# hypre-space/hypredrive

Measured on NVIDIA B200. Metric: AMG-PCG solve DOF-iters/s, 7pt Poisson 256^3 per GPU, higher is better.
Workload: dtype f64

## Files before the change

### hypredrive_b200/csrc/hdk_amg_setup.cu

```cuda
#include "hdk_amg.cuh"
#include <algorithm>
#include <math.h>
#include <stdlib.h>
#include <time.h>

namespace hdk {

#define C_PT 1
#define F_PT -1
#define SF_PT -3

static double g_t_last = 0.0;
static bool   g_timing = false;
static double wall_now()
{
   struct timespec ts;
   clock_gettime(CLOCK_MONOTONIC, &ts);
   return (double)ts.tv_sec + 1e-9 * (double)ts.tv_nsec;
}
static void stage_mark(const char *name, int level)
{
   if (!g_timing) return;
   cudaStreamSynchronize(g.stream);
   double t = wall_now();
// ... 1640 lines not shown
{
   int i = blockIdx.x * blockDim.x + threadIdx.x;
   if (i >= n) return;
   int    b = rp[i], e = rp[i + 1];
   double d = e > b ? val[b] : 0.0, v;
   if (option == 1)
   {
      v = 0.0;
      for (int k = b; k < e; k++) v = __dadd_rn(v, fabs(val[k]));
      if (orp) for (int k = orp[i]; k < orp[i + 1]; k++) v = __dadd_rn(v, fabs(oval[k]));
      if (d < 0) v = -v;
   }
   else if (option == 4)
   {
      double od = 0.0;
      if (orp) for (int k = orp[i]; k < orp[i + 1]; k++) od = __dadd_rn(od, fabs(oval[k]));
      v = __dadd_rn(fabs(d), __dmul_rn(0.5, od));
      if (v <= (4.0 / 3.0) * fabs(d)) v = fabs(d);
      if (d < 0) v = -v;
   }
   else v = d;
   l1[i] = v;
}

static int relax_l1_option(int type)
{
   if (type == 18) return 1;
   if (type == 8 || type == 13 || type == 14) return 4;
   return 5;
}

static int build_l1(const hdk_csr_s &A, int option, double **out)
{
   int n = A.diag.nrows;
   HDK_TRY(dalloc(out, (size_t)n + 8));
   const int    *orp = A.offd.nnz > 0 ? A.offd.rowptr : nullptr;
   const double *ov  = A.offd.nnz > 0 ? A.offd.val : nullptr;
   k_l1<<<cdiv(n, 256), 256, 0, g.stream>>>(A.diag.rowptr, A.diag.val, orp, ov, n, option, *out);
   HDK_LAUNCH_CHECK();
   return HDK_OK;
}

template <bool FILL>
__global__ void k_lower(const int *rp, const int *col, const double *val, int n, int *cnt, const int *lrp, int *lcol, double *lval)
{
   int i = blockIdx.x * blockDim.x + threadIdx.x;
   if (i > n) return;
   if (i == n) { if (!FILL) cnt[n] = 0; return; }
   int c = 0, p = FILL ? lrp[i] : 0;
   for (int k = rp[i]; k < rp[i + 1]; k++)
      if (col[k] < i) { if (FILL) { lcol[p] = col[k]; lval[p] = val[k]; p++; } else c++; }
   if (!FILL) cnt[i] = c;
}

static int build_lower(const DevCSR &A, DevCSR &L)
{
   int  n = A.nrows;
   int *cnt, *lrp;
   HDK_TRY(dalloc(&cnt, (size_t)n + 1));
   HDK_TRY(dalloc(&lrp, (size_t)n + 1));
   k_lower<false><<<cdiv(n + 1, 256), 256, 0, g.stream>>>(A.rowptr, A.col, A.val, n, cnt, nullptr, nullptr, nullptr);
   HDK_LAUNCH_CHECK();
   HDK_TRY(exclusive_scan_int(cnt, lrp, n + 1));
   int nnz = 0;
   HDK_CUDA(cudaMemcpyAsync(&nnz, lrp + n, sizeof(int), cudaMemcpyDeviceToHost, g.stream));
   HDK_CUDA(cudaStreamSynchronize(g.stream));
   dfree(cnt);
   HDK_TRY(csr_alloc(L, n, n, nnz));
   dfree(L.rowptr); L.rowptr = lrp;
   k_lower<true><<<cdiv(n + 1, 256), 256, 0, g.stream>>>(A.rowptr, A.col, A.val, n, nullptr, lrp, L.col, L.val);
   HDK_LAUNCH_CHECK();
   return csr_analyze(L);
}

__global__ void k_dense_fill(const int *rp, const int *col, const double *val, int n, double *M )
{
   int i = blockIdx.x * blockDim.x + threadIdx.x;
   if (i >= n) return;
   for (int k = rp[i]; k < rp[i + 1]; k++) M[(size_t)i * 2 * n + col[k]] += val[k];
   M[(size_t)i * 2 * n + n + i] = 1.0;
}

__global__ void __launch_bounds__(1024) k_gauss_jordan(double *M, int n, double *inv)
{
   __shared__ double sval[32];
   __shared__ int    sidx[32];
   __shared__ int    piv;
   __shared__ double pivval;
   const int tid = threadIdx.x, nt = blockDim.x, w = 2 * n;
   for (int k = 0; k < n; k++)
   {
      double best = -1.0; int bi = k;
      for (int r = k + tid; r < n; r += nt) { double v = fabs(M[(size_t)r * w + k]); if (v > best) { best = v; bi = r; } }
      for (int o = 16; o > 0; o >>= 1)
      {
         double ov = __shfl_down_sync(0xffffffffu, best, o); int oi = __shfl_down_sync(0xffffffffu, bi, o);
         if (ov > best || (ov == best && oi < bi)) { best = ov; bi = oi; }
      }
      if ((tid & 31) == 0) { sval[tid >> 5] = best; sidx[tid >> 5] = bi; }
      __syncthreads();
      if (tid == 0)
      {
         double b = sval[0]; int i2 = sidx[0];
         for (int q = 1; q < (nt + 31) / 32; q++) if (sval[q] > b || (sval[q] == b && sidx[q] < i2)) { b = sval[q]; i2 = sidx[q]; }
         piv = i2; pivval = M[(size_t)i2 * w + k];
      }
      __syncthreads();
      int    pr = piv;
      double pv = pivval;
      if (pv != 0.0)
      {
         if (pr != k)
            for (int j = tid; j < w; j += nt) { double t = M[(size_t)k * w + j]; M[(size_t)k * w + j] = M[(size_t)pr * w + j]; M[(size_t)pr * w + j] = t; }
         __syncthreads();
         for (int j = tid; j < w; j += nt) M[(size_t)k * w + j] /= pv;
         __syncthreads();
         for (int idx = tid; idx < n * w; idx += nt)
         {
            int r = idx / w, j = idx - r * w;
            if (r != k && j != k)
            {
               double f = M[(size_t)r * w + k];
               if (f != 0.0) M[(size_t)r * w + j] -= f * M[(size_t)k * w + j];
            }
         }
         __syncthreads();
         for (int r = tid; r < n; r += nt) if (r != k) M[(size_t)r * w + k] = 0.0;
      }
      __syncthreads();
   }
   for (int idx = tid; idx < n * n; idx += nt) { int r = idx / n, j = idx - r * n; inv[idx] = M[(size_t)r * w + n + j]; }
}

constexpr int GJ_ONE_CTA = 1024;
__global__ void __launch_bounds__(1024) k_gj_pivot(double *M, int n, int k, double *f)
{
   __shared__ double sval[32];
   __shared__ int    sidx[32];
   __shared__ int    piv;
   __shared__ double pivval;
   const int tid = threadIdx.x, nt = blockDim.x, w = 2 * n;
   double best = -1.0; int bi = k;
   for (int r = k + tid; r < n; r += nt) { double v = fabs(M[(size_t)r * w + k]); if (v > best) { best = v; bi = r; } }
   for (int o = 16; o > 0; o >>= 1)
   {
      double ov = __shfl_down_sync(0xffffffffu, best, o); int oi = __shfl_down_sync(0xffffffffu, bi, o);
      if (ov > best || (ov == best && oi < bi)) { best = ov; bi = oi; }
   }
   if ((tid & 31) == 0) { sval[tid >> 5] = best; sidx[tid >> 5] = bi; }
   __syncthreads();
   if (tid == 0)
   {
      double b = sval[0]; int i2 = sidx[0];
      for (int q = 1; q < (nt + 31) / 32; q++) if (sval[q] > b || (sval[q] == b && sidx[q] < i2)) { b = sval[q]; i2 = sidx[q]; }
      piv = i2; pivval = M[(size_t)i2 * w + k];
   }
   __syncthreads();
   const int    pr = piv;
   const double pv = pivval;
   if (pv != 0.0)
   {
      if (pr != k)
         for (int j = tid; j < w; j += nt) { double t = M[(size_t)k * w + j]; M[(size_t)k * w + j] = M[(size_t)pr * w + j]; M[(size_t)pr * w + j] = t; }
      __syncthreads();
      for (int j = tid; j < w; j += nt) M[(size_t)k * w + j] /= pv;
   }
   for (int r = tid; r < n; r += nt) f[r] = (pv != 0.0 && r != k) ? M[(size_t)r * w + k] : 0.0;
}

__global__ void k_gj_eliminate(double *M, int n, int k, const double *f)
{
   const int    r = blockIdx.y, w = 2 * n;
   const double fr = f[r];
   if (fr == 0.0) return;
   for (int j = k + blockIdx.x * blockDim.x + threadIdx.x; j < w; j += gridDim.x * blockDim.x)
   {
      if (j == k) M[(size_t)r * w + k] = 0.0;
      else M[(size_t)r * w + j] -= fr * M[(size_t)k * w + j];
   }
}

__global__ void k_gj_extract(const double *M, int n, double *inv)
{
   const int64_t idx = blockIdx.x * (int64_t)blockDim.x + threadIdx.x;
   if (idx >= (int64_t)n * n) return;
   const int64_t r = idx / n, j = idx - r * n;
   inv[idx] = M[r * 2 * n + n + j];
}

static int build_dense_inverse(const DevCSR &A, double **inv)
{
   int     n = A.nrows;
   double *M;
   HDK_TRY(dalloc(&M, (size_t)n * 2 * n + 8));
   if (int rc = dalloc(inv, (size_t)n * n + 8)) { dfree(M); return rc; }
   HDK_CUDA(cudaMemsetAsync(M, 0, sizeof(double) * ((size_t)n * 2 * n), g.stream));
   k_dense_fill<<<cdiv(n, 128), 128, 0, g.stream>>>(A.rowptr, A.col, A.val, n, M);
   HDK_LAUNCH_CHECK();
   if (n <= GJ_ONE_CTA)
   {
      k_gauss_jordan<<<1, 1024, 0, g.stream>>>(M, n, *inv);
      HDK_LAUNCH_CHECK();
   }
   else
   {
      double *f;
      if (int rc = dalloc(&f, (size_t)n + 8)) { dfree(M); return rc; }
      for (int k = 0; k < n; k++)
      {
         k_gj_pivot<<<1, 1024, 0, g.stream>>>(M, n, k, f);
         k_gj_eliminate<<<dim3(cdiv(2 * n - k, 256), n), 256, 0, g.stream>>>(M, n, k, f);
      }
      HDK_LAUNCH_CHECK();
      k_gj_extract<<<(unsigned)(((int64_t)n * n + 255) / 256), 256, 0, g.stream>>>(M, n, *inv);
      HDK_LAUNCH_CHECK();
      dfree(f);
   }
   dfree(M);
   return HDK_OK;
}

hdk_csr_s *wrap_local(DevCSR &D, int64_t grows)
{
   hdk_csr_s *A  = new hdk_csr_s();
   A->row_start  = 0; A->row_end = (int64_t)D.nrows - 1; A->global_rows = grows; A->global_nnz = D.nnz;
   A->diag       = D;
   D             = DevCSR();
   return A;
}

void destroy_local(hdk_csr_s *A)
{
   if (!A) return;
   csr_free(A->diag); csr_free(A->offd);
   halo_plan_free(A->halo);
   dfree(A->offd_rows);
   delete A;
}

}

using namespace hdk;

extern "C" {

void hdk_amg_default_params(hdk_amg_params *p)
{
   p->coarsen_type = 8; p->strong_th = 0.25; p->max_row_sum = 0.9;
   p->max_coarse_size = 64; p->min_coarse_size = 0; p->max_levels = 25;
   p->interp_type = 6; p->max_nnz_row = 4; p->trunc_factor = 0.0;
   p->relax_down = 18; p->relax_up = 18; p->relax_coarse = 9;
   p->sweeps_down = p->sweeps_up = p->sweeps_coarse = 1;
   p->relax_weight = p->outer_weight = 1.0;
   p->rand_seed = 2747; p->keep_transpose = 1; p->print_level = 0;
}

int hdk_amg_destroy(hdk_amg *M)
{
   if (!M) return HDK_OK;
   if (g.inited)
   {
      for (auto &L : M->lev)
      {
         if (L.owns_A) destroy_local(L.A);
         destroy_local(L.P); destroy_local(L.R);
         csr_free(L.S); csr_free(L.L);
         dfree(L.cf); dfree(L.measure); dfree(L.f2c);
         if (L.l1_up != L.l1_down) dfree(L.l1_up);
         dfree(L.l1_down);
         dfree(L.u); dfree(L.f); dfree(L.t); dfree(L.gs1); dfree(L.gs2);
         for (int w = 0; w < 2; w++) { dfree(L.dbg_ip[w]); dfree(L.dbg_col[w]); dfree(L.dbg_val[w]); }
      }
      dfree(M->ge_inv); dfree(M->full_f); dfree(M->full_u);
      ipc_gather_free(M->gather);
      for (auto &G : M->graphs) if (G.exec) cudaGraphExecDestroy((cudaGraphExec_t)G.exec);
      M->graphs.clear();
   }
   if (M->tail) hdk_amg_destroy(M->tail);
   delete M;
   return HDK_OK;
}

int finalize_levels(hdk_amg_s *M, const hdk_amg_params *prm, int64_t live_max_rows)
{
   int    rc = HDK_OK;
   double bytes = 0.0;
   for (int l = 0; l < M->nlev && rc == HDK_OK; l++)
   {
      AmgLevel &L = M->lev[(size_t)l];
      int       n = L.n;
      if (live_max_rows >= 0 && n > live_max_rows) continue;
      if ((rc = build_l1(*L.A, relax_l1_option(prm->relax_down), &L.l1_down))) break;
      if (relax_l1_option(prm->relax_up) == relax_l1_option(prm->relax_down)) L.l1_up = L.l1_down;
      else if ((rc = build_l1(*L.A, relax_l1_option(prm->relax_up), &L.l1_up))) break;
      if ((rc = dalloc(&L.t, (size_t)n + 8))) break;
      if (l > 0)
      {
         if ((rc = dalloc(&L.u, (size_t)n + 8))) break;
         if ((rc = dalloc(&L.f, (size_t)n + 8))) break;
      }
      bool tsgs = (prm->relax_down == 11 || prm->relax_down == 12 || prm->relax_up == 11 || prm->relax_up == 12);
      if (tsgs && (rc = build_lower(L.A->diag, L.L))) break;
      if (tsgs && ((rc = dalloc(&L.gs1, (size_t)n + 8)) || (rc = dalloc(&L.gs2, (size_t)n + 8)))) break;
      double nnzA = (double)L.A->diag.nnz + L.A->offd.nnz;
      if (L.P)
      {
         double nnzP = (double)L.P->diag.nnz + L.P->offd.nnz, ncl = (double)L.P->diag.ncols;
         bytes += 24.0 * n;
         bytes += 12.0 * nnzA + 4.0 * (n + 1) + 24.0 * n;
         bytes += 12.0 * nnzP + 4.0 * (ncl + 1) + 8.0 * n + 8.0 * ncl;
         bytes += 12.0 * nnzP + 4.0 * (n + 1) + 16.0 * n + 8.0 * ncl;
         bytes += 12.0 * nnzA + 4.0 * (n + 1) + 32.0 * n;
      }
      else bytes += 8.0 * (double)n * n + 16.0 * n;
   }
   M->vcycle_bytes = bytes;
   return rc;
}

int setup_serial(const hdk_csr_s *A0, const hdk_amg_params *prm, hdk_amg_s **out, bool keep_f2c,
                 int64_t live_max_rows)
{
   hdk_amg_s *M = new hdk_amg_s();
   M->prm       = *prm;
   M->keep_f2c  = keep_f2c;
   M->keep_debug = tune_amg_keep_debug();
   int rc       = HDK_OK;
   M->lev.emplace_back();
   M->lev[0].A = const_cast<hdk_csr_s *>(A0);
   M->lev[0].owns_A = false;
   M->lev[0].n = A0->diag.nrows;
   int  level = 0;
   bool more  = prm->max_levels > 1;
   double nnz0 = (double)A0->diag.nnz + A0->offd.nnz, nnz_sum = nnz0;
   while (more && rc == HDK_OK)
   {
      AmgLevel        &L = M->lev[(size_t)level];
      const hdk_csr_s &A = *L.A;
      int              n = L.n;
      stage_mark(nullptr, level);
      if ((rc = build_strength(A, prm->strong_th, prm->max_row_sum, L.S))) break;
      stage_mark("strength", level);
      if ((rc = dalloc(&L.cf, (size_t)n + 1))) break;
      double *meas, *keep = nullptr;
      if ((rc = dalloc(&meas, (size_t)n + 1))) break;
      if (M->keep_debug) { if ((rc = dalloc(&keep, (size_t)n + 1))) break; }
      L.measure = keep;
      int64_t goff = (level == 0) ? A.row_start : 0;
      rc = run_pmis(L.S, prm->rand_seed, goff, L.cf, meas, keep, nullptr);
      stage_mark("pmis", level);
      dfree(meas);
      if (rc) break;
      int *flag, *f2c;
      if ((rc = dalloc(&flag, (size_t)n + 1))) break;
      if ((rc = dalloc(&f2c, (size_t)n + 1))) break;
      k_cf_flag<<<cdiv(n + 1, 256), 256, 0, g.stream>>>(L.cf, n, flag);
      g.launches++;
      if ((rc = exclusive_scan_int(flag, f2c, n + 1))) break;
      int nc = 0;
      cudaMemcpyAsync(&nc, f2c + n, sizeof(int), cudaMemcpyDeviceToHost, g.stream);
      cudaStreamSynchronize(g.stream);
      dfree(flag);
      if (nc == 0 || nc == n || nc < prm->min_coarse_size) { dfree(f2c); break; }
      DevCSR P, R, C;
      rc = build_interp(A.diag, L.S, L.cf, f2c, nc, prm->max_nnz_row, prm->trunc_factor, P, -1, -1);
      stage_mark("interp", level);
      if (keep_f2c) L.f2c = f2c; else dfree(f2c);
      if (rc) break;
      if ((rc = csr_transpose(P, R))) break;
      stage_mark("transpose", level);
      if ((rc = build_rap(R, A.diag, P, C, -1, -1))) break;
      stage_mark("rap", level);
      C.coarse_op = true;
      if (live_max_rows < 0 || n <= live_max_rows)
      {
         if ((rc = csr_analyze(P))) break;
         if ((rc = csr_analyze(R))) break;
      }
      if (live_max_rows < 0 || nc <= live_max_rows)
      {
         if ((rc = csr_analyze(C))) break;
      }
      stage_mark("analyze", level);
      nnz_sum += C.nnz;
      L.P = wrap_local(P, n);
      L.R = wrap_local(R, nc);
      M->lev.emplace_back();
      AmgLevel &N = M->lev.back();
      N.A = wrap_local(C, nc); N.owns_A = true; N.n = nc;
      level++;
      if (level == prm->max_levels - 1 || nc <= prm->max_coarse_size) more = false;
      if (!M->keep_debug) csr_free(M->lev[(size_t)level - 1].S);
   }
   if (rc == HDK_OK)
   {
      M->nlev = level + 1;
      M->op_complexity = nnz_sum / (nnz0 > 0 ? nnz0 : 1.0);
      rc = finalize_levels(M, prm, live_max_rows);
   }
   if (rc == HDK_OK)
   {
      AmgLevel &Lc = M->lev[(size_t)M->nlev - 1];
      bool      want_ge = (prm->relax_coarse == 9 || prm->relax_coarse == 99 || prm->relax_coarse == 19);
      if (want_ge && (double)Lc.n * Lc.n < 2.0e8 && Lc.n > 0 && Lc.A->offd.nnz == 0)
      {
         rc = build_dense_inverse(Lc.A->diag, &M->ge_inv);
         M->ge_n = Lc.n;
      }
   }
   if (rc == HDK_OK) rc = (cudaStreamSynchronize(g.stream) == cudaSuccess) ? HDK_OK : set_error(HDK_ERR_CUDA, "setup sync failed: %s", cudaGetErrorString(cudaGetLastError()));
   if (rc != HDK_OK) { hdk_amg_destroy(M); return rc; }
   *out = M;
   return HDK_OK;
}

__global__ void k_shift_i64(const int64_t *in, int64_t *out, int64_t n, int64_t shift)
{
   int64_t i = blockIdx.x * (int64_t)blockDim.x + threadIdx.x;
   if (i < n) out[i] = in[i] + shift;
}
__global__ void k_slice_indptr(const int *rp, int r0, int n, int64_t *out)
{
   int i = blockIdx.x * blockDim.x + threadIdx.x;
   if (i <= n) out[i] = (int64_t)rp[r0 + i] - (int64_t)rp[r0];
}
__global__ void k_slice_entries(const int *col, const double *val, int64_t k0, int64_t cnt, int64_t *ocol, double *oval)
{
   int64_t k = blockIdx.x * (int64_t)blockDim.x + threadIdx.x;
   if (k < cnt) { ocol[k] = col[k0 + k]; oval[k] = val[k0 + k]; }
}

static int slice_rows(const DevCSR &D, int r0, int r1, int64_t cs, int64_t ce, int64_t grows, int64_t gcols,
                      bool square, bool distributed, hdk_csr_s **out)
{
   int      n = r1 - r0;
   int      k[2];
   HDK_CUDA(cudaMemcpyAsync(&k[0], D.rowptr + r0, sizeof(int), cudaMemcpyDeviceToHost, g.stream));
   HDK_CUDA(cudaMemcpyAsync(&k[1], D.rowptr + r1, sizeof(int), cudaMemcpyDeviceToHost, g.stream));
   HDK_CUDA(cudaStreamSynchronize(g.stream));
   int64_t  cnt = (int64_t)k[1] - k[0];
   int64_t *ip, *cj;
   double  *va;
   HDK_TRY(dalloc(&ip, (size_t)n + 1));
   HDK_TRY(dalloc(&cj, (size_t)cnt + 1));
   HDK_TRY(dalloc(&va, (size_t)cnt + 1));
   k_slice_indptr<<<cdiv(n + 1, 256), 256, 0, g.stream>>>(D.rowptr, r0, n, ip);
   HDK_LAUNCH_CHECK();
   if (cnt > 0)
   {
      k_slice_entries<<<cdiv(cnt, 256), 256, 0, g.stream>>>(D.col, D.val, k[0], cnt, cj, va);
      HDK_LAUNCH_CHECK();
   }
   int rc = parcsr_build(r0, (int64_t)r1 - 1, cs, ce, grows, gcols, square, distributed, false, ip, cj, va, out);
   dfree(ip); dfree(cj); dfree(va);
   return rc;
}

static int setup_distributed(const hdk_csr_s *A0, const hdk_amg_params *prm, hdk_amg_s **out)
{
   const int R = g.nranks, me = g.rank;
   stage_mark(nullptr, -2);
   if (!A0->orig_indptr) return set_error(HDK_ERR_INVALID, "distributed setup needs the matrix to be built at N > 1");
   std::vector<int64_t> rows_all, nnz_all;
   HDK_TRY(allgather_i64_host(A0->diag.nrows, rows_all));
   HDK_TRY(allgather_i64_host(A0->orig_nnz, nnz_all));
   std::vector<int64_t> roff((size_t)R + 1, 0), koff((size_t)R + 1, 0);
   for (int r = 0; r < R; r++) { roff[(size_t)r + 1] = roff[(size_t)r] + rows_all[(size_t)r]; koff[(size_t)r + 1] = koff[(size_t)r] + nnz_all[(size_t)r]; }
   const int64_t N = roff[(size_t)R], NNZ = koff[(size_t)R];
   if (N > 2000000000LL || NNZ > 2000000000LL)
      return set_error(HDK_ERR_UNSUPPORTED, "global problem (%lld rows, %lld nnz) exceeds the int32 limits of the replicated setup", (long long)N, (long long)NNZ);
   if (roff[(size_t)me] != A0->row_start) return set_error(HDK_ERR_INVALID, "row partition is not contiguous in rank order");
   int64_t *gip, *gcj;
   double  *gva;
   HDK_TRY(dalloc(&gip, (size_t)N + 1));
   HDK_TRY(dalloc(&gcj, (size_t)NNZ + 1));
   HDK_TRY(dalloc(&gva, (size_t)NNZ + 1));
   {
      int64_t n = rows_all[(size_t)me];
      k_shift_i64<<<cdiv(n, 256), 256, 0, g.stream>>>(A0->orig_indptr, gip + roff[(size_t)me], n, koff[(size_t)me]);
      HDK_LAUNCH_CHECK();
      HDK_CUDA(cudaMemcpyAsync(gcj + koff[(size_t)me], A0->orig_cols, sizeof(int64_t) * (size_t)A0->orig_nnz, cudaMemcpyDeviceToDevice, g.stream));
      HDK_CUDA(cudaMemcpyAsync(gva + koff[(size_t)me], A0->orig_vals, sizeof(double) * (size_t)A0->orig_nnz, cudaMemcpyDeviceToDevice, g.stream));
      HDK_CUDA(cudaMemcpyAsync(gip + N, &NNZ, sizeof(int64_t), cudaMemcpyHostToDevice, g.stream));
   }
   for (int r = 0; r < R; r++)
   {
      HDK_TRY(bcast_bytes(gip + roff[(size_t)r], sizeof(int64_t) * (size_t)rows_all[(size_t)r], r));
      HDK_TRY(bcast_bytes(gcj + koff[(size_t)r], sizeof(int64_t) * (size_t)nnz_all[(size_t)r], r));
      HDK_TRY(bcast_bytes(gva + koff[(size_t)r], sizeof(double) * (size_t)nnz_all[(size_t)r], r));
   }
   const int64_t rep_rows = tune_replicate_rows();
   hdk_csr_s *G = nullptr;
   int rc = parcsr_build(0, N - 1, 0, N - 1, N, N, true, false, false, gip, gcj, gva, &G, N <= rep_rows);
   dfree(gip); dfree(gcj); dfree(gva);
   if (rc) return rc;
   stage_mark("gather A", -2);
   hdk_amg_s *Mg = nullptr;
   g_share = !(getenv("HDK_SETUP_SHARE") && atoi(getenv("HDK_SETUP_SHARE")) == 0);
   if (getenv("HDK_SHARE_MIN_ROWS")) g_share_min_rows = atoi(getenv("HDK_SHARE_MIN_ROWS"));
   rc = setup_serial(G, prm, &Mg, true, rep_rows);
   g_share = false;
   if (rc) { destroy_local(G); return rc; }
   Mg->lev[0].owns_A = true;
   stage_mark("global setup", -2);
   const int nl = Mg->nlev;
   std::vector<std::vector<int64_t>> starts((size_t)nl);
   starts[0] = roff;
   int tail_level = nl - 1;
   for (int l = 0; l < nl; l++)
   {
      bool empty = false;
      for (int r = 0; r < R; r++) if (starts[(size_t)l][(size_t)r + 1] <= starts[(size_t)l][(size_t)r]) empty = true;
      if (Mg->lev[(size_t)l].n <= rep_rows || empty) { tail_level = l; break; }
      if (l + 1 < nl)
      {
         std::vector<int64_t> nxt((size_t)R + 1, 0);
         for (int r = 0; r <= R; r++)
         {
            int v = 0;
            HDK_CUDA(cudaMemcpyAsync(&v, Mg->lev[(size_t)l].f2c + starts[(size_t)l][(size_t)r], sizeof(int), cudaMemcpyDeviceToHost, g.stream));
            HDK_CUDA(cudaStreamSynchronize(g.stream));
            nxt[(size_t)r] = v;
         }
         starts[(size_t)l + 1] = nxt;
      }
   }
   hdk_amg_s *M = new hdk_amg_s();
   M->prm = *prm;
   M->tail = Mg; M->tail_level = tail_level;
   M->op_complexity = Mg->op_complexity;
   for (int l = 0; l < tail_level && rc == HDK_OK; l++)
   {
      AmgLevel &Lg = Mg->lev[(size_t)l];
      M->lev.emplace_back();
      AmgLevel &L = M->lev.back();
      const int64_t fs = starts[(size_t)l][(size_t)me], fe = starts[(size_t)l][(size_t)me + 1];
      const int64_t cs = starts[(size_t)l + 1][(size_t)me], ce = starts[(size_t)l + 1][(size_t)me + 1];
      const int64_t nf = Lg.n, nc = Mg->lev[(size_t)l + 1].n;
      L.n = (int)(fe - fs);
      if (l == 0) { L.A = const_cast<hdk_csr_s *>(A0); L.owns_A = false; }
      else
      {
         if ((rc = slice_rows(Lg.A->diag, (int)fs, (int)fe, fs, fe - 1, nf, nf, true, true, &L.A))) break;
         L.owns_A = true;
      }
      if (l + 1 < tail_level)
      {
         if ((rc = slice_rows(Lg.P->diag, (int)fs, (int)fe, cs, ce - 1, nf, nc, false, true, &L.P))) break;
      }
      else
      {
         if ((rc = slice_rows(Lg.P->diag, (int)fs, (int)fe, 0, nc - 1, nf, nc, false, false, &L.P))) break;
      }
      if ((rc = slice_rows(Lg.R->diag, (int)cs, (int)ce, fs, fe - 1, nc, nf, false, true, &L.R))) break;
   }
   stage_mark("slice", -2);
   if (rc == HDK_OK)
   {
      M->nlev = tail_level;
      M->tail_n   = Mg->lev[(size_t)tail_level].n;
      M->tail_off = starts[(size_t)tail_level][(size_t)me];
      M->tail_cnt = starts[(size_t)tail_level][(size_t)me + 1] - M->tail_off;
      rc = finalize_levels(M, prm, -1);
      double vb = M->vcycle_bytes;
      for (int l = tail_level; l < nl; l++)
      {
         AmgLevel &Lg = Mg->lev[(size_t)l];
         double    n = Lg.n, nnzA = Lg.A->diag.nnz;
         if (Lg.P) { double nnzP = Lg.P->diag.nnz, ncl = Lg.P->diag.ncols; vb += 24.0 * n + 2 * (12.0 * nnzA + 4.0 * n) + 56.0 * n + 2 * (12.0 * nnzP) + 28.0 * n + 16.0 * ncl; }
         else vb += 8.0 * n * n + 16.0 * n;
      }
      M->vcycle_bytes = vb;
   }
   if (rc == HDK_OK) rc = dalloc(&M->full_f, (size_t)M->tail_n + 8);
   if (rc == HDK_OK) rc = dalloc(&M->full_u, (size_t)M->tail_n + 8);
   if (rc == HDK_OK)
   {
      for (int l = 0; l < tail_level; l++)
      {
         AmgLevel &Lg = Mg->lev[(size_t)l];
         if (Lg.owns_A) { destroy_local(Lg.A); Lg.A = nullptr; Lg.owns_A = false; }
         destroy_local(Lg.P); Lg.P = nullptr;
         destroy_local(Lg.R); Lg.R = nullptr;
         csr_free(Lg.S); csr_free(Lg.L);
         dfree(Lg.cf); Lg.cf = nullptr; dfree(Lg.measure); Lg.measure = nullptr; dfree(Lg.f2c); Lg.f2c = nullptr;
         if (Lg.l1_up != Lg.l1_down) dfree(Lg.l1_up);
         dfree(Lg.l1_down); Lg.l1_down = Lg.l1_up = nullptr;
         dfree(Lg.u); dfree(Lg.f); dfree(Lg.t); Lg.u = Lg.f = Lg.t = nullptr;
      }
      HDK_CUDA(cudaStreamSynchronize(g.stream));
   }
   stage_mark("finalize", -2);
   if (rc != HDK_OK) { hdk_amg_destroy(M); return rc; }
   *out = M;
   return HDK_OK;
}

int hdk_amg_setup(const hdk_csr *A0, const hdk_amg_params *prm, hdk_amg **out)
{
   HDK_TRY(require_init());
   if (!A0 || !prm || !out) return set_error(HDK_ERR_INVALID, "hdk_amg_setup: null argument");
   if (prm->interp_type != 6) return set_error(HDK_ERR_UNSUPPORTED, "interpolation type %d: only extended+i (6) has a device kernel", prm->interp_type);
   if (prm->trunc_factor < 0.0 || prm->trunc_factor >= 1.0) return set_error(HDK_ERR_INVALID, "interpolation trunc_factor must be in [0, 1)");
   g_timing = getenv("HDK_SETUP_TIMING") && atoi(getenv("HDK_SETUP_TIMING")) == 1;
   const bool replicated = getenv("HDK_SETUP_REPLICATED") && atoi(getenv("HDK_SETUP_REPLICATED")) == 1;
   const bool force_dist = getenv("HDK_SETUP_DIST_FORCE") && atoi(getenv("HDK_SETUP_DIST_FORCE")) == 1;
   if (g.nranks > 1 && replicated) return setup_distributed(A0, prm, out);
   if (g.nranks > 1 || (force_dist && A0->orig_indptr)) return setup_distributed_rows(A0, prm, out);
   return setup_serial(A0, prm, out, false, -1);
}

int hdk_amg_num_levels(const hdk_amg *M) { return M ? M->nlev + (M->tail ? M->tail->nlev - M->tail_level : 0) : 0; }
int hdk_amg_num_dist_levels(const hdk_amg *M) { return (M && M->tail) ? M->nlev : 0; }
double hdk_amg_operator_complexity(const hdk_amg *M) { return M ? M->op_complexity : 0.0; }
double hdk_amg_vcycle_bytes(const hdk_amg *M) { return M ? M->vcycle_bytes : 0.0; }

static const hdk_amg_s *resolve_level(const hdk_amg *M, int &level)
{
   if (M && M->tail && level >= M->nlev) { level = level - M->nlev + M->tail_level; return M->tail; }
   return M;
}

int hdk_amg_level_info(const hdk_amg *M, int level, int64_t *rows, int64_t *nnz_A, int64_t *nnz_P)
{
   M = resolve_level(M, level);
   if (!M || level < 0 || level >= M->nlev) return set_error(HDK_ERR_INVALID, "level out of range");
   const AmgLevel &L = M->lev[(size_t)level];
   if (rows) *rows = L.n;
   if (nnz_A) *nnz_A = (int64_t)L.A->diag.nnz + L.A->offd.nnz;
   if (nnz_P) *nnz_P = L.P ? L.P->diag.nnz : 0;
   return HDK_OK;
}

int hdk_amg_get_matrix(const hdk_amg *M, int level, int which, int32_t *rowptr_h, int32_t *col_h, double *val_h)
{
   HDK_TRY(require_init());
   M = resolve_level(M, level);
   if (!M || level < 0 || level >= M->nlev) return set_error(HDK_ERR_INVALID, "level out of range");
   const AmgLevel &L = M->lev[(size_t)level];
   const DevCSR   *D = nullptr;
   if (which == 0) D = &L.A->diag;
   else if (which == 1 && L.P) D = &L.P->diag;
   else if (which == 2 && L.R) D = &L.R->diag;
   else if (which == 3 && L.S.rowptr) D = &L.S;
   if (!D) return set_error(HDK_ERR_INVALID, "matrix %d not available on level %d", which, level);
   if (rowptr_h) HDK_CUDA(cudaMemcpyAsync(rowptr_h, D->rowptr, sizeof(int) * ((size_t)D->nrows + 1), cudaMemcpyDeviceToHost, g.stream));
   if (col_h && D->nnz) HDK_CUDA(cudaMemcpyAsync(col_h, D->col, sizeof(int) * (size_t)D->nnz, cudaMemcpyDeviceToHost, g.stream));
   if (val_h && D->val && D->nnz) HDK_CUDA(cudaMemcpyAsync(val_h, D->val, sizeof(double) * (size_t)D->nnz, cudaMemcpyDeviceToHost, g.stream));
   HDK_CUDA(cudaStreamSynchronize(g.stream));
   return HDK_OK;
}

static int get_level_array(const hdk_amg *M, int level, const void *src, size_t bytes, void *dst)
{
   HDK_TRY(require_init());
   if (!M || level < 0 || level >= M->nlev || !src) return set_error(HDK_ERR_INVALID, "array not available on level %d", level);
   return hdk_copy_d2h(dst, src, bytes);
}
int hdk_amg_get_cf(const hdk_amg *M, int level, int32_t *cf_h)
{
   M = resolve_level(M, level);
   if (!M || level < 0 || level >= M->nlev) return set_error(HDK_ERR_INVALID, "level out of range");
   return get_level_array(M, level, M->lev[(size_t)level].cf, sizeof(int) * (size_t)M->lev[(size_t)level].n, cf_h);
}
int hdk_amg_get_measure(const hdk_amg *M, int level, double *m_h)
{
   M = resolve_level(M, level);
   if (!M || level < 0 || level >= M->nlev) return set_error(HDK_ERR_INVALID, "level out of range");
   return get_level_array(M, level, M->lev[(size_t)level].measure, sizeof(double) * (size_t)M->lev[(size_t)level].n, m_h);
}
int hdk_amg_get_l1(const hdk_amg *M, int level, double *l1_h)
{
   M = resolve_level(M, level);
   if (!M || level < 0 || level >= M->nlev) return set_error(HDK_ERR_INVALID, "level out of range");
   return get_level_array(M, level, M->lev[(size_t)level].l1_down, sizeof(double) * (size_t)M->lev[(size_t)level].n, l1_h);
}

int hdk_amg_strength(const hdk_csr *A, double theta, double max_row_sum, int64_t *nnz_S, int32_t **rowptr_d, int32_t **col_d)
{
   HDK_TRY(require_init());
   if (!A) return set_error(HDK_ERR_INVALID, "null matrix");
   DevCSR S;
   HDK_TRY(build_strength(*A, theta, max_row_sum, S));
   *nnz_S = S.nnz; *rowptr_d = S.rowptr; *col_d = S.col;
   return HDK_OK;
}

int hdk_amg_pmis(int64_t n, const int32_t *S_rowptr_d, const int32_t *S_col_d, int seed, int64_t global_offset,
                 int32_t *cf_d, double *measure_d, int *iterations)
{
   HDK_TRY(require_init());
   DevCSR S;
   S.nrows = (int)n; S.ncols = (int)n; S.rowptr = const_cast<int *>(S_rowptr_d); S.col = const_cast<int *>(S_col_d);
   HDK_CUDA(cudaMemcpyAsync(&S.nnz, S_rowptr_d + n, sizeof(int), cudaMemcpyDeviceToHost, g.stream));
   HDK_CUDA(cudaStreamSynchronize(g.stream));
   double *work;
   HDK_TRY(dalloc(&work, (size_t)n + 1));
   int rc = run_pmis(S, seed, global_offset, cf_d, work, measure_d, iterations);
   dfree(work);
   return rc;
}

}
```

### hypredrive_b200/csrc/hdk_amg_solve.cu

```cuda
#include "hdk_amg.cuh"

namespace hdk {

__global__ void __launch_bounds__(256) k_dense_apply(const double *__restrict__ Ainv, const double *__restrict__ f,
                                                     double *__restrict__ u, int n)
{
   int row = blockIdx.x * 8 + (threadIdx.x >> 5), lane = threadIdx.x & 31;
   if (row >= n) return;
   double acc = 0.0;
   for (int j = lane; j < n; j += 32) acc += Ainv[(size_t)row * n + j] * f[j];
   acc = warp_sum(acc);
   if (lane == 0) u[row] = acc;
}

static bool is_jacobi(int t) { return t == 18 || t == 7 || t == 0; }

static int relax_sweep(hdk_amg_s *M, int l, int type, const double *l1, const double *f, const double *in,
                       double *out, int fin, double *fin_out, const hdk_csr_s *export_to = nullptr)
{
   AmgLevel &L = M->lev[(size_t)l];
   SpmvArgs  a;
   a.x = in; a.y = out; a.b = f; a.d = l1; a.w = M->prm.relax_weight;
   if (is_jacobi(type))
   {
// ... 59 lines not shown
      HDK_LAUNCH_CHECK();
      return HDK_OK;
   }
   int     type = (M->prm.relax_coarse == 9 || M->prm.relax_coarse == 99) ? 18 : M->prm.relax_coarse;
   double *cur = u, *oth = alt;
   int     sweeps = M->prm.sweeps_coarse < 1 ? 1 : M->prm.sweeps_coarse;
   for (int s = 0; s < sweeps; s++)
   {
      if (s == 0 && zero_guess && is_jacobi(type))
      {
         HDK_TRY(vec_scaled_div(cur, f, L.l1_down, M->prm.relax_weight, L.n));
      }
      else
      {
         if (s == 0 && zero_guess) HDK_TRY(vec_fill(cur, 0.0, L.n));
         HDK_TRY(relax_sweep(M, l, type, L.l1_down, f, cur, oth, FIN_NONE, nullptr));
         double *tmp = cur; cur = oth; oth = tmp;
      }
   }
   *result = cur;
   return HDK_OK;
}

static double *cycle_start_buffer(hdk_amg_s *M, int l0, double *u0, bool zero_guess)
{
   const hdk_amg_params &p = M->prm;
   const int nfine = M->tail ? M->nlev : M->nlev - 1;
   int       oop;
   if (nfine <= l0) oop = 0;
   else
   {
      int down_oop = zero_guess && is_jacobi(p.relax_down) ? (p.sweeps_down > 0 ? p.sweeps_down - 1 : 0) : p.sweeps_down;
      oop          = down_oop + p.sweeps_up;
   }
   const bool start_in_u0 = zero_guess ? (oop % 2 == 0) : true;
   return start_in_u0 ? u0 : M->lev[(size_t)l0].t;
}

static int amg_cycle_impl(hdk_amg_s *M, const double *f0, double *u0, bool zero_guess, int fin, double *fin_out, int l0, int kg);

static int first_graph_level(hdk_amg_s *M, int l0)
{
   if (M->tail || M->graph_off) return -1;
   const int64_t rows = tune_graph_rows();
   if (rows <= 0) return -1;
   const hdk_amg_params &p = M->prm;
   if (!is_jacobi(p.relax_down) || !is_jacobi(p.relax_up)) return -1;
   for (int l = l0; l < M->nlev; l++)
      if (M->lev[(size_t)l].n <= rows) return l;
   return -1;
}

static int cycle_graph_run(hdk_amg_s *M, const double *f, double *u, bool zero_guess, bool prefilled, int kg)
{
   for (auto &G : M->graphs)
      if (G.f == f && G.u == u && G.zero_guess == zero_guess && G.prefilled == prefilled && G.level == kg)
      {
         HDK_CUDA(cudaGraphLaunch((cudaGraphExec_t)G.exec, g.stream));
         g.launches += G.nodes;
         return HDK_OK;
      }
   const int64_t before = g.launches;
   cudaGraph_t   graph = nullptr;
   if (cudaStreamBeginCapture(g.stream, cudaStreamCaptureModeThreadLocal) != cudaSuccess)
   {
      cudaGetLastError();
      M->graph_off = true;
      M->prefilled_at = prefilled ? kg : -1;
      return amg_cycle_impl(M, f, u, zero_guess, FIN_NONE, nullptr, kg, -1);
   }
   M->prefilled_at = prefilled ? kg : -1;
   int         rc = amg_cycle_impl(M, f, u, zero_guess, FIN_NONE, nullptr, kg, -1);
   cudaError_t e = cudaStreamEndCapture(g.stream, &graph);
   cudaGraphExec_t exec = nullptr;
   if (rc == HDK_OK && e == cudaSuccess && graph) e = cudaGraphInstantiate(&exec, graph, 0);
   if (graph) cudaGraphDestroy(graph);
   if (rc != HDK_OK || e != cudaSuccess || !exec)
   {
      cudaGetLastError();
      M->graph_off = true;
      if (rc != HDK_OK) return rc;
      M->prefilled_at = prefilled ? kg : -1;
      return amg_cycle_impl(M, f, u, zero_guess, FIN_NONE, nullptr, kg, -1);
   }
   hdk_amg_s::CycleGraph G;
   G.f = f; G.u = u; G.zero_guess = zero_guess; G.prefilled = prefilled; G.level = kg; G.exec = exec;
   G.nodes = (int)(g.launches - before);
   g.launches = before;
   M->graphs.push_back(G);
   HDK_CUDA(cudaGraphLaunch(exec, g.stream));
   g.launches += G.nodes;
   return HDK_OK;
}

int amg_cycle(hdk_amg_s *M, const double *f0, double *u0, bool zero_guess, int fin, double *fin_out, int l0)
{
   int kg = first_graph_level(M, l0);
   if (kg == l0)
   {
      if (fin == FIN_NONE)
      {
         const bool pf = (M->prefilled_at == l0) && zero_guess;
         M->prefilled_at = -1;
         return cycle_graph_run(M, f0, u0, zero_guess, pf, l0);
      }
      kg = (l0 + 1 < M->nlev) ? l0 + 1 : -1;
   }
   return amg_cycle_impl(M, f0, u0, zero_guess, fin, fin_out, l0, kg);
}

static int amg_cycle_impl(hdk_amg_s *M, const double *f0, double *u0, bool zero_guess, int fin, double *fin_out, int l0, int kg)
{
   const int             nl = M->nlev;
   const bool            has_tail = (M->tail != nullptr);
   const int             nfine = has_tail ? nl : nl - 1;
   const hdk_amg_params &p = M->prm;
   std::vector<double *> cur((size_t)nl + 1, nullptr), alt((size_t)nl + 1, nullptr);
   std::vector<const double *> rhs((size_t)nl + 1, nullptr);
   bool                  fin_done = false;
   if (has_tail && nl == 0)
   {
      HDK_TRY(vec_fill(M->full_f, 0.0, M->tail_n));
      HDK_TRY(vec_copy(M->full_f + M->tail_off, f0, M->tail_cnt));
      HDK_TRY(allreduce_dev(M->full_f, (int)M->tail_n));
      if (!zero_guess)
      {
         HDK_TRY(vec_fill(M->full_u, 0.0, M->tail_n));
         HDK_TRY(vec_copy(M->full_u + M->tail_off, u0, M->tail_cnt));
         HDK_TRY(allreduce_dev(M->full_u, (int)M->tail_n));
      }
      HDK_TRY(amg_cycle(M->tail, M->full_f, M->full_u, zero_guess, FIN_NONE, nullptr, M->tail_level));
      HDK_TRY(vec_copy(u0, M->full_u + M->tail_off, M->tail_cnt));
      if (fin != FIN_NONE) HDK_TRY(vec_dot_dev(f0, u0, M->tail_cnt, fin, fin_out));
      return HDK_OK;
   }
   {
      AmgLevel &L0 = M->lev[(size_t)l0];
      cur[(size_t)l0] = cycle_start_buffer(M, l0, u0, zero_guess);
      alt[(size_t)l0] = (cur[(size_t)l0] == u0) ? L0.t : u0;
      rhs[(size_t)l0] = f0;
   }
   for (int l = l0 + 1; l < nl; l++) { cur[(size_t)l] = M->lev[(size_t)l].u; alt[(size_t)l] = M->lev[(size_t)l].t; rhs[(size_t)l] = M->lev[(size_t)l].f; }

   bool prefilled = (M->prefilled_at == l0) && zero_guess;
   M->prefilled_at = -1;
   const bool sub = (kg > l0 && kg < nl);
   const int  ndown = sub ? kg : nfine;
   if (sub) cur[(size_t)kg] = cycle_start_buffer(M, kg, M->lev[(size_t)kg].u, true);
   for (int l = l0; l < ndown; l++)
   {
      AmgLevel &L = M->lev[(size_t)l];
      bool      zg = (l > l0) || zero_guess;
      for (int s = 0; s < p.sweeps_down; s++)
      {
         if (s == 0 && zg && is_jacobi(p.relax_down))
         {
            tl_mark(l, 5);
            if (!prefilled) HDK_TRY(vec_scaled_div(cur[(size_t)l], rhs[(size_t)l], L.l1_down, p.relax_weight, L.n, L.A));
         }
         else
         {
            tl_mark(l, 10);
            if (s == 0 && zg) HDK_TRY(vec_fill(cur[(size_t)l], 0.0, L.n));
            HDK_TRY(relax_sweep(M, l, p.relax_down, L.l1_down, rhs[(size_t)l], cur[(size_t)l], alt[(size_t)l], FIN_NONE, nullptr, L.A));
            std::swap(cur[(size_t)l], alt[(size_t)l]);
         }
      }
      if (p.sweeps_down == 0 && zg) HDK_TRY(vec_fill(cur[(size_t)l], 0.0, L.n));
      if (p.sweeps_down == 0 && zg)
      {
         HDK_TRY(vec_copy(alt[(size_t)l], rhs[(size_t)l], L.n));
      }
      else
      {
         SpmvArgs a;
         a.x = cur[(size_t)l]; a.y = alt[(size_t)l]; a.b = rhs[(size_t)l];
         a.export_to = L.R;
         tl_mark(l, 1);
         HDK_TRY(parcsr_matvec(*L.A, SPMV_RESIDUAL, a));
      }
      SpmvArgs rr;
      tl_mark(l, 2);
      rr.x = alt[(size_t)l];
      prefilled = false;
      if (l + 1 < nl) rr.y = M->lev[(size_t)l + 1].f;
      else
      {
         if (M->gather.on) rr.y = ipc_gather_buffer(M->gather) + M->tail_off;
         else
         {
            HDK_TRY(vec_fill(M->full_f, 0.0, M->tail_n));
            rr.y = M->full_f + M->tail_off;
         }
      }
      if (l + 1 < nfine && p.sweeps_down > 0 && is_jacobi(p.relax_down))
      {
         rr.y2 = cur[(size_t)l + 1]; rr.d = M->lev[(size_t)l + 1].l1_down; rr.w = p.relax_weight;
         if (!(sub && l + 1 == kg)) { rr.export_to = M->lev[(size_t)l + 1].A; rr.export_y2 = true; }
         HDK_TRY(parcsr_matvec(*L.R, SPMV_SET_DIV, rr));
         prefilled = true;
      }
      else HDK_TRY(parcsr_matvec(*L.R, SPMV_SET, rr));
   }
   const double *coarse_sol = nullptr;
   tl_mark(ndown, 6);
   if (sub)
   {
      AmgLevel &Lk = M->lev[(size_t)kg];
      HDK_TRY(cycle_graph_run(M, Lk.f, Lk.u, true, prefilled, kg));
      cur[(size_t)kg] = Lk.u;
   }
   else if (has_tail)
   {
      const double *tf = M->full_f;
      if (M->gather.on)
      {
         HDK_TRY(ipc_gather(M->gather, M->tail_off, M->tail_cnt));
         tf = M->gather.buf[M->gather.seq & 1];
      }
      else HDK_TRY(allreduce_dev(M->full_f, (int)M->tail_n));
      HDK_TRY(amg_cycle(M->tail, tf, M->full_u, true, FIN_NONE, nullptr, M->tail_level));
      coarse_sol = M->full_u;
   }
   else
   {
      const int Lc = nl - 1;
      double   *res;
      bool      zg = (Lc > l0) || zero_guess;
      HDK_TRY(coarse_solve(M, Lc, rhs[(size_t)Lc], cur[(size_t)Lc], alt[(size_t)Lc], zg, &res));
      if (res != cur[(size_t)Lc]) std::swap(cur[(size_t)Lc], alt[(size_t)Lc]);
      coarse_sol = cur[(size_t)Lc];
   }
   for (int l = ndown - 1; l >= l0; l--)
   {
      AmgLevel &L = M->lev[(size_t)l];
      tl_mark(l, 3);
      SpmvArgs a;
      a.x = (l + 1 < nl) ? cur[(size_t)l + 1] : coarse_sol;
      a.y = cur[(size_t)l];
      if (p.sweeps_up > 0) a.export_to = L.A;
      else if (l > l0) a.export_to = M->lev[(size_t)l - 1].P;
      HDK_TRY(parcsr_matvec(*L.P, SPMV_ADD, a));
      for (int s = 0; s < p.sweeps_up; s++)
      {
         bool last = (l == l0 && s == p.sweeps_up - 1);
         int  f_   = (last && fin != FIN_NONE) ? fin : FIN_NONE;
         const hdk_csr_s *next = (s + 1 < p.sweeps_up) ? L.A : (l > l0 ? M->lev[(size_t)l - 1].P : nullptr);
         tl_mark(l, 4);
         HDK_TRY(relax_sweep(M, l, p.relax_up, L.l1_up, rhs[(size_t)l], cur[(size_t)l], alt[(size_t)l], f_, fin_out, next));
         std::swap(cur[(size_t)l], alt[(size_t)l]);
         if (f_ != FIN_NONE) fin_done = true;
      }
   }
   tl_mark(l0, 0);
   if (cur[(size_t)l0] != u0) HDK_TRY(vec_copy(u0, cur[(size_t)l0], M->lev[(size_t)l0].n));
   if (fin != FIN_NONE && !fin_done) HDK_TRY(vec_dot_dev(f0, u0, M->lev[(size_t)l0].n, fin, fin_out));
   return HDK_OK;
}

bool amg_prefill_target(hdk_amg_s *M, double *z, double **buf, const double **d, double *w, const hdk_csr_s **reader)
{
   if (reader) *reader = (M->nlev > 0) ? M->lev[0].A : nullptr;
   const hdk_amg_params &p = M->prm;
   const bool has_tail = (M->tail != nullptr);
   const int  nl = M->nlev, nfine = has_tail ? nl : nl - 1;
   if (nl == 0 || nfine <= 0 || p.sweeps_down <= 0 || !is_jacobi(p.relax_down)) return false;
   const int  oop = (p.sweeps_down - 1) + p.sweeps_up;
   *buf = (oop % 2 == 0) ? z : M->lev[0].t;
   *d   = M->lev[0].l1_down;
   *w   = p.relax_weight;
   return true;
}

int amg_precond(hdk_amg_s *M, const double *r, double *z, int fin, double *fin_out)
{
   return amg_cycle(M, r, z, true, fin, fin_out, 0);
}

}

using namespace hdk;

extern "C" {

int hdk_amg_apply(hdk_amg *M, const double *r_d, double *z_d)
{
   HDK_TRY(require_init());
   if (!M) return set_error(HDK_ERR_INVALID, "null hierarchy");
   return amg_precond(M, r_d, z_d, FIN_NONE, nullptr);
}

int hdk_amg_vcycle(hdk_amg *M, const double *f_d, double *u_d)
{
   HDK_TRY(require_init());
   if (!M) return set_error(HDK_ERR_INVALID, "null hierarchy");
   return amg_cycle(M, f_d, u_d, false, FIN_NONE, nullptr, 0);
}

int hdk_time_kernel(const hdk_csr *A, hdk_amg *M, int kernel, int reps, double *avg_ms, double *bytes)
{
   HDK_TRY(require_init());
   if (!A) return set_error(HDK_ERR_INVALID, "null matrix");
   const int64_t n = A->diag.nrows;
   const double  nnz = (double)A->diag.nnz + A->offd.nnz;
   double *x, *y, *b, *d, *z;
   HDK_TRY(dalloc(&x, (size_t)n + 8)); HDK_TRY(dalloc(&y, (size_t)n + 8));
   HDK_TRY(dalloc(&b, (size_t)n + 8)); HDK_TRY(dalloc(&d, (size_t)n + 8));
   HDK_TRY(dalloc(&z, (size_t)n + 8));
   HDK_TRY(hdk_vec_random(x, n, A->row_start, 1));
   HDK_TRY(hdk_vec_random(b, n, A->row_start, 2));
   HDK_TRY(vec_fill(d, 6.0, n));
   HDK_TRY(vec_fill(y, 0.0, n));
   double by = 0.0;
   int    rc = HDK_OK;
   for (int pass = 0; pass < 2 && rc == HDK_OK; pass++)
   {
      int count = pass == 0 ? 3 : reps;
      if (pass == 1) HDK_CUDA(cudaEventRecord(g.ev_a, g.stream));
      for (int it = 0; it < count && rc == HDK_OK; it++)
      {
         SpmvArgs a;
         a.x = x; a.y = y; a.b = b; a.d = d;
         switch (kernel)
         {
            case 0: rc = parcsr_matvec(*A, SPMV_SET, a); by = 12.0 * nnz + 4.0 * (n + 1) + 16.0 * n; break;
            case 1: rc = parcsr_matvec(*A, SPMV_JACOBI, a); by = 12.0 * nnz + 4.0 * (n + 1) + 32.0 * n; break;
            case 2: rc = parcsr_matvec(*A, SPMV_RESIDUAL, a); by = 12.0 * nnz + 4.0 * (n + 1) + 24.0 * n; break;
            case 3:
               rc = vec_fill(g.dscal + S_ALPHA, 1e-3, 1);
               if (rc == HDK_OK) rc = pcg_update_xr(y, b, x, d, n, g.dscal, FIN_IPROD, nullptr, z, d, 1.0);
               by = 64.0 * n; break;
            case 5:
               rc = vec_fill(g.dscal + S_BETA, 0.5, 1);
               if (rc == HDK_OK) rc = pcg_update_p(y, x, n, g.dscal);
               by = 24.0 * n; break;
            case 4:
               if (!M) rc = set_error(HDK_ERR_INVALID, "V-cycle timing needs a hierarchy");
               else { rc = amg_precond(M, b, y, FIN_NONE, nullptr); by = M->vcycle_bytes; }
               break;
            case 6:
               if (!M || M->nlev < 1 || !M->lev[0].L.rowptr) rc = set_error(HDK_ERR_INVALID, "two-stage GS timing needs a hierarchy set up with relaxation 11 or 12");
               else
               {
                  const int    type = (M->prm.relax_down == 12 || M->prm.relax_up == 12) ? 12 : 11;
                  const double nnzL = (double)M->lev[0].L.nnz;
                  rc = relax_sweep(M, 0, type, M->lev[0].l1_down, b, x, y, FIN_NONE, nullptr);
                  by = 12.0 * nnz + 4.0 * (n + 1) + 40.0 * n + (type == 11 ? 1 : 2) * (12.0 * nnzL + 4.0 * (n + 1) + 32.0 * n) + (type == 12 ? 8.0 * n : 0.0);
               }
               break;
            case 7: rc = halo_exchange_begin(*A, x); by = 8.0 * A->halo.n_send; break;
            case 8:
               dbg_skip_exchange(true);
               rc = parcsr_matvec(*A, SPMV_SET, a); by = 12.0 * nnz + 4.0 * (n + 1) + 16.0 * n;
               dbg_skip_exchange(false);
               break;
            default: rc = set_error(HDK_ERR_INVALID, "unknown kernel id %d", kernel);
         }
      }
   }
   if (rc == HDK_OK)
   {
      HDK_CUDA(cudaEventRecord(g.ev_b, g.stream));
      HDK_CUDA(cudaEventSynchronize(g.ev_b));
      float ms = 0.f;
      HDK_CUDA(cudaEventElapsedTime(&ms, g.ev_a, g.ev_b));
      if (avg_ms) *avg_ms = (double)ms / (reps > 0 ? reps : 1);
      if (bytes) *bytes = by;
   }
   dfree(x); dfree(y); dfree(b); dfree(d); dfree(z);
   return rc;
}

}
```

### hypredrive_b200/csrc/hdk_csr.cu

```cuda
#include "hdk_internal.cuh"
#include <cub/cub.cuh>

namespace hdk {

__global__ void k_split_count(const int64_t *indptr, const int64_t *cols, int nrows, int64_t rs,
                              int64_t re, int *cnt_d, int *cnt_o)
{
   int r = blockIdx.x * blockDim.x + threadIdx.x;
   if (r > nrows) return;
   if (r == nrows) { cnt_d[r] = 0; cnt_o[r] = 0; return; }
   int cd = 0, co = 0;
   for (int64_t k = indptr[r]; k < indptr[r + 1]; k++)
   {
      int64_t c = cols[k];
      if (c >= rs && c <= re) cd++; else co++;
   }
   cnt_d[r] = cd; cnt_o[r] = co;
}

__global__ void k_split_fill(const int64_t *indptr, const int64_t *cols, const double *vals, int nrows,
                             int64_t rs, int64_t re, const int *rp_d, int *col_d, double *val_d,
                             const int *rp_o, int64_t *gcol_o, double *val_o, int square)
{
   int r = blockIdx.x * blockDim.x + threadIdx.x;
// ... 304 lines not shown
   return HDK_OK;
}

__global__ void k_offd_correct(const int *rows, const int *rowptr, const int *col, const double *val, int nrows,
                               const double *xh, double *y, const double *d, double w, int mode,
                               double alpha, const double *dotv, const double *diag_part,
                               double *dot_out, double *partials, unsigned *ticket)
{
   __shared__ double red[128 / 32];
   __shared__ int    lastflag;
   double            dcorr = 0.0;
   int i = blockIdx.x * blockDim.x + threadIdx.x;
   if (i < nrows)
   {
      int r = rows[i];
      int s = rowptr[r], e = rowptr[r + 1];
      double acc = 0.0;
      for (int k = s; k < e; k++) acc += val[k] * __ldcg(xh + col[k]);
      double delta = 0.0;
      switch (mode)
      {
         case SPMV_SET:
         case SPMV_ADD: delta = acc; break;
         case SPMV_AXPBY: delta = alpha * acc; break;
         case SPMV_RESIDUAL: delta = -acc; break;
         case SPMV_JACOBI:
         case SPMV_JACOBI_R: { double dd = d[r]; if (dd != 0.0) delta = -(w * acc) / dd; break; }
      }
      y[r] += delta;
      if (dotv) dcorr = dotv[r] * delta;
   }
   if (dotv)
   {
      double bs = block_sum<128>(dcorr, red);
      if (threadIdx.x == 0)
      {
         partials[blockIdx.x] = bs;
         __threadfence();
         unsigned t = atomicInc(ticket, gridDim.x - 1);
         lastflag   = (t == gridDim.x - 1);
      }
      __syncthreads();
      if (lastflag)
      {
         __threadfence();
         double sacc = 0.0;
         for (unsigned b = threadIdx.x; b < gridDim.x; b += 128) sacc += __ldcg(partials + b);
         __syncthreads();
         sacc = block_sum<128>(sacc, red);
         if (threadIdx.x == 0) *dot_out = *diag_part + sacc;
      }
   }
}

__device__ __forceinline__ void grid_xyz(int64_t row, int nx, int ny, int &gx, int &gy, int &gz)
{
   gx = (int)(row % nx);
   int64_t t = row / nx;
   gy = (int)(t % ny);
   gz = (int)(t / ny);
}

__device__ __forceinline__ double axial_velocity(double y, double z, double Hy, double Hz, double umax)
{
   return 16.0 * umax * (y / Hy) * (1.0 - y / Hy) * (z / Hz) * (1.0 - z / Hz);
}

__global__ void k_stencil_count(int kind, int nx, int ny, int nz, int64_t rs, int nrows, int64_t *cnt)
{
   int i = blockIdx.x * blockDim.x + threadIdx.x;
   if (i > nrows) return;
   if (i == nrows) { cnt[i] = 0; return; }
   int gx, gy, gz;
   grid_xyz(rs + i, nx, ny, gx, gy, gz);
   int c;
   if (kind == 27)
   {
      int ax = 1 + (gx > 0) + (gx < nx - 1), ay = 1 + (gy > 0) + (gy < ny - 1), az = 1 + (gz > 0) + (gz < nz - 1);
      c = ax * ay * az;
   }
   else c = 1 + (gx > 0) + (gx < nx - 1) + (gy > 0) + (gy < ny - 1) + (gz > 0) + (gz < nz - 1);
   cnt[i] = c;
}

__global__ void k_stencil_fill(int kind, int nx, int ny, int nz, double c0, double c1, double c2,
                               int64_t rs, int nrows, const int64_t *indptr, int64_t *cols, double *vals,
                               double *b)
{
   int i = blockIdx.x * blockDim.x + threadIdx.x;
   if (i >= nrows) return;
   int64_t row = rs + i;
   int gx, gy, gz;
   grid_xyz(row, nx, ny, gx, gy, gz);
   int64_t p = indptr[i];
   const int64_t sx = 1, sy = nx, sz = (int64_t)nx * ny;
   if (kind == 7)
   {
      cols[p] = row; vals[p++] = 2.0 * (c0 + c1 + c2);
      if (gz > 0) { cols[p] = row - sz; vals[p++] = -c2; }
      if (gy > 0) { cols[p] = row - sy; vals[p++] = -c1; }
      if (gx > 0) { cols[p] = row - sx; vals[p++] = -c0; }
      if (gx < nx - 1) { cols[p] = row + sx; vals[p++] = -c0; }
      if (gy < ny - 1) { cols[p] = row + sy; vals[p++] = -c1; }
      if (gz < nz - 1) { cols[p] = row + sz; vals[p++] = -c2; }
      if (b) b[i] = (gy == 0) ? 1.0 : 0.0;
   }
   else if (kind == 27)
   {
      double center = 0.0;
      for (int dz = -1; dz <= 1; dz++)
         for (int dy = -1; dy <= 1; dy++)
            for (int dx = -1; dx <= 1; dx++)
            {
               if (!dx && !dy && !dz) continue;
               int    ndiff = (dx != 0) + (dy != 0) + (dz != 0);
               double adj   = 0.0;
               if (dx) adj += c0 / ndiff;
               if (dy) adj += c1 / ndiff;
               if (dz) adj += c2 / ndiff;
               int x = gx + dx, y = gy + dy, z = gz + dz;
               if (x >= 0 && x < nx && y >= 0 && y < ny && z >= 0 && z < nz)
               {
                  cols[p] = row + dx * sx + dy * sy + dz * sz; vals[p++] = -adj;
               }
               center += adj;
            }
      cols[p] = row; vals[p++] = center;
      if (b) b[i] = (gy == 0) ? 1.0 : 0.0;
   }
   else
   {
      const double Lx = 4.0, Ly = 1.0, Lz = 1.0;
      const double hx = Lx / nx, hy = Ly / ny, hz = Lz / nz;
      const double vol = hx * hy * hz;
      const double Dx = c0 * hy * hz / hx, Dy = c0 * hx * hz / hy, Dz = c0 * hx * hy / hz;
      const double Ax = hy * hz;
      double z = ((double)gz + 0.5) * hz, y = ((double)gy + 0.5) * hy;
      double Cf = axial_velocity(y, z, Ly, Lz, c1) * Ax;
      double Cf_pos = Cf > 0.0 ? Cf : 0.0, Cf_neg = Cf < 0.0 ? -Cf : 0.0;
      int64_t dpos = p++;
      double  diag = vol / c2, rhs = 0.0;
      cols[dpos] = row;
      if (gx > 0) { diag += Dx + Cf_neg; cols[p] = row - sx; vals[p++] = -(Dx + Cf_pos); }
      else { diag += 2.0 * Dx + Cf_neg; rhs = (2.0 * Dx + Cf_pos) * 1.0; }
      if (gx < nx - 1) { diag += Dx + Cf_pos; cols[p] = row + sx; vals[p++] = -(Dx + Cf_neg); }
      else diag += Cf_pos;
      if (gy > 0) { diag += Dy; cols[p] = row - sy; vals[p++] = -Dy; }
      if (gy < ny - 1) { diag += Dy; cols[p] = row + sy; vals[p++] = -Dy; }
      if (gz > 0) { diag += Dz; cols[p] = row - sz; vals[p++] = -Dz; }
      if (gz < nz - 1) { diag += Dz; cols[p] = row + sz; vals[p++] = -Dz; }
      vals[dpos] = diag;
      if (b) b[i] = rhs;
   }
}

int wait_globals_csr(long long tmo, int *err)
{
   return wait_globals_set(tmo, err) == cudaSuccess ? HDK_OK : set_error(HDK_ERR_CUDA, "cannot set the wait budget");
}

}

using namespace hdk;

extern "C" {

int hdk_csr_from_device(int64_t row_start, int64_t row_end, int64_t global_rows, const int64_t *indptr_d,
                        const int64_t *cols_d, const double *vals_d, hdk_csr **A)
{
   HDK_TRY(require_init());
   return parcsr_from_device(row_start, row_end, global_rows, indptr_d, cols_d, vals_d, A);
}

int hdk_csr_from_host(int64_t row_start, int64_t row_end, int64_t global_rows, const int64_t *indptr_h,
                      const int64_t *cols_h, const double *vals_h, hdk_csr **A)
{
   HDK_TRY(require_init());
   if (!indptr_h) return set_error(HDK_ERR_INVALID, "indptr is NULL");
   if (row_end < row_start) return set_error(HDK_ERR_INVALID, "invalid row range");
   int64_t n = row_end - row_start + 1;
   int64_t k0 = indptr_h[0], k1 = indptr_h[n];
   if (k0 < 0 || k1 < k0) return set_error(HDK_ERR_INVALID, "indptr must be nonnegative and nondecreasing");
   int64_t nnz = k1 - k0;
   if (nnz > 0 && (!cols_h || !vals_h)) return set_error(HDK_ERR_INVALID, "col_indices/data are NULL");
   if (nnz > 2000000000LL) return set_error(HDK_ERR_UNSUPPORTED, "local nnz exceeds int32");
   int64_t *ip, *cj;
   double  *va;
   HDK_TRY(dalloc(&ip, (size_t)n + 1));
   HDK_TRY(dalloc(&cj, (size_t)nnz + 1));
   HDK_TRY(dalloc(&va, (size_t)nnz + 1));
   std::vector<int64_t> shifted((size_t)n + 1);
   for (int64_t i = 0; i <= n; i++)
   {
      shifted[(size_t)i] = indptr_h[i] - k0;
      if (i > 0 && indptr_h[i] < indptr_h[i - 1])
      {
         dfree(ip); dfree(cj); dfree(va);
         return set_error(HDK_ERR_INVALID, "indptr must be nondecreasing");
      }
   }
   HDK_CUDA(cudaMemcpyAsync(ip, shifted.data(), sizeof(int64_t) * ((size_t)n + 1), cudaMemcpyHostToDevice, g.stream));
   if (nnz > 0)
   {
      HDK_CUDA(cudaMemcpyAsync(cj, cols_h + k0, sizeof(int64_t) * (size_t)nnz, cudaMemcpyHostToDevice, g.stream));
      HDK_CUDA(cudaMemcpyAsync(va, vals_h + k0, sizeof(double) * (size_t)nnz, cudaMemcpyHostToDevice, g.stream));
   }
   HDK_CUDA(cudaStreamSynchronize(g.stream));
   int rc = parcsr_from_device(row_start, row_end, global_rows, ip, cj, va, A);
   dfree(ip); dfree(cj); dfree(va);
   return rc;
}

int hdk_csr_stencil(int kind, int nx, int ny, int nz, const double c[3], int64_t row_start, int64_t row_end,
                    hdk_csr **A, double *b_d)
{
   HDK_TRY(require_init());
   if (kind != 7 && kind != 27 && kind != 107) return set_error(HDK_ERR_INVALID, "unknown stencil kind %d", kind);
   int64_t N = (int64_t)nx * ny * nz;
   if (row_start < 0 || row_end >= N || row_end < row_start) return set_error(HDK_ERR_INVALID, "row range outside the grid");
   int      n = (int)(row_end - row_start + 1);
   int64_t *cnt, *ip;
   HDK_TRY(dalloc(&cnt, (size_t)n + 1));
   HDK_TRY(dalloc(&ip, (size_t)n + 1));
   k_stencil_count<<<cdiv(n + 1, 256), 256, 0, g.stream>>>(kind, nx, ny, nz, row_start, n, cnt);
   HDK_LAUNCH_CHECK();
   HDK_TRY(exclusive_scan_i64_i64(cnt, ip, (int64_t)n + 1));
   int64_t nnz = 0;
   HDK_CUDA(cudaMemcpyAsync(&nnz, ip + n, sizeof(int64_t), cudaMemcpyDeviceToHost, g.stream));
   HDK_CUDA(cudaStreamSynchronize(g.stream));
   dfree(cnt);
   int64_t *cols;
   double  *vals;
   HDK_TRY(dalloc(&cols, (size_t)nnz + 1));
   HDK_TRY(dalloc(&vals, (size_t)nnz + 1));
   k_stencil_fill<<<cdiv(n, 256), 256, 0, g.stream>>>(kind, nx, ny, nz, c[0], c[1], c[2], row_start, n, ip, cols, vals, b_d);
   HDK_LAUNCH_CHECK();
   int rc = parcsr_from_device(row_start, row_end, N, ip, cols, vals, A);
   dfree(ip); dfree(cols); dfree(vals);
   return rc;
}

int hdk_csr_destroy(hdk_csr *A)
{
   if (!A) return HDK_OK;
   if (g.inited)
   {
      csr_free(A->diag); csr_free(A->offd);
      halo_plan_free(A->halo);
      dfree(A->orig_indptr); dfree(A->orig_cols); dfree(A->orig_vals); dfree(A->offd_rows);
   }
   delete A;
   return HDK_OK;
}

int hdk_csr_info(const hdk_csr *A, int64_t *local_rows, int64_t *global_rows, int64_t *local_nnz, int64_t *global_nnz)
{
   if (!A) return set_error(HDK_ERR_INVALID, "null matrix");
   if (local_rows) *local_rows = A->diag.nrows;
   if (global_rows) *global_rows = A->global_rows;
   if (local_nnz) *local_nnz = (int64_t)A->diag.nnz + A->offd.nnz;
   if (global_nnz) *global_nnz = A->global_nnz;
   return HDK_OK;
}

int hdk_csr_get_diag(const hdk_csr *A, int32_t *rowptr_h, int32_t *col_h, double *val_h)
{
   HDK_TRY(require_init());
   if (!A) return set_error(HDK_ERR_INVALID, "null matrix");
   if (rowptr_h) HDK_CUDA(cudaMemcpyAsync(rowptr_h, A->diag.rowptr, sizeof(int) * ((size_t)A->diag.nrows + 1), cudaMemcpyDeviceToHost, g.stream));
   if (col_h && A->diag.nnz) HDK_CUDA(cudaMemcpyAsync(col_h, A->diag.col, sizeof(int) * (size_t)A->diag.nnz, cudaMemcpyDeviceToHost, g.stream));
   if (val_h && A->diag.nnz) HDK_CUDA(cudaMemcpyAsync(val_h, A->diag.val, sizeof(double) * (size_t)A->diag.nnz, cudaMemcpyDeviceToHost, g.stream));
   HDK_CUDA(cudaStreamSynchronize(g.stream));
   return HDK_OK;
}

int hdk_csr_matvec(const hdk_csr *A, double alpha, const double *x_d, double beta, double *y_d)
{
   HDK_TRY(require_init());
   if (!A) return set_error(HDK_ERR_INVALID, "null matrix");
   SpmvArgs a;
   a.x = x_d; a.y = y_d; a.alpha = alpha; a.beta = beta;
   if (alpha == 1.0 && beta == 0.0) return parcsr_matvec(*A, SPMV_SET, a);
   return parcsr_matvec(*A, SPMV_AXPBY, a);
}

int hdk_csr_residual(const hdk_csr *A, const double *x_d, const double *b_d, double *r_d)
{
   HDK_TRY(require_init());
   if (!A) return set_error(HDK_ERR_INVALID, "null matrix");
   SpmvArgs a;
   a.x = x_d; a.y = r_d; a.b = b_d;
   return parcsr_matvec(*A, SPMV_RESIDUAL, a);
}

int hdk_csr_spmv_kind(const hdk_csr *A, int *kind, double *avg_row, int *max_row)
{
   if (!A) return set_error(HDK_ERR_INVALID, "null matrix");
   if (kind) *kind = A->diag.kind;
   if (avg_row) *avg_row = A->diag.avg_row;
   if (max_row) *max_row = A->diag.max_row;
   return HDK_OK;
}

}
```

### hypredrive_b200/csrc/hdk_internal.cuh

```cuda
#pragma once
#include <cuda_runtime.h>
#include <stdint.h>
#include <stdio.h>
#include <string.h>
#include <string>
#include <vector>
#include "hdk.h"

namespace hdk {

struct Ctx
{
   bool         inited = false;
   int          device = 0;
   int          sm_count = 148;
   cudaStream_t stream = nullptr;
   cudaStream_t comm_stream = nullptr;
   cudaEvent_t  ev_a = nullptr, ev_b = nullptr, ev_scal = nullptr, ev_halo = nullptr, ev_pack = nullptr;
   int          rank = 0, nranks = 1;
   void        *nccl = nullptr;
   int64_t      launches = 0;
   double      *partials = nullptr;
   unsigned    *counters = nullptr;
   double      *dscal = nullptr;
   double      *hscal = nullptr;
   char         err[1024] = {0};
};

extern Ctx g;
constexpr int PARTIALS_CAP = 1 << 20;

int  set_error(int code, const char *fmt, ...);
int  require_init();

#define HDK_CUDA(call)                                                                     \
   do {                                                                                    \
      cudaError_t e__ = (call);                                                            \
      if (e__ != cudaSuccess)                                                              \
         return hdk::set_error(HDK_ERR_CUDA, "%s:%d %s -> %s", __FILE__, __LINE__, #call,  \
                               cudaGetErrorString(e__));                                   \
   } while (0)

#define HDK_TRY(call)                  \
   do {                                \
      int rc__ = (call);               \
      if (rc__ != HDK_OK) return rc__; \
   } while (0)

#define HDK_LAUNCH_CHECK()                                                                  \
   do {                                                                                     \
      hdk::g.launches++;                                                                    \
      cudaError_t e__ = cudaGetLastError();                                                 \
      if (e__ != cudaSuccess)                                                               \
         return hdk::set_error(HDK_ERR_CUDA, "%s:%d launch -> %s", __FILE__, __LINE__,      \
                               cudaGetErrorString(e__));                                    \
   } while (0)

template <class T>
inline int dalloc(T **p, size_t n)
{
   *p = nullptr;
   if (n == 0) n = 1;
   cudaError_t e = cudaMallocAsync((void **)p, n * sizeof(T), g.stream);
   if (e != cudaSuccess)
      return set_error(HDK_ERR_ALLOC, "cudaMallocAsync(%zu bytes) -> %s", n * sizeof(T),
                       cudaGetErrorString(e));
   return HDK_OK;
}
inline void dfree(void *p)
{
   if (p) cudaFreeAsync(p, g.stream);
}

inline int cdiv(int64_t a, int64_t b) { return (int)((a + b - 1) / b); }

struct DevCSR
{
   int     nrows = 0, ncols = 0;
   int     nnz = 0;
   int    *rowptr = nullptr;
   int    *col = nullptr;
   double *val = nullptr;
   int     kind = 0;
   int     max_row = 0;
   double  avg_row = 0.0;
   int     tgt = 0, cap = 0;
   int     lpr = 1;
   int     nblk = 0;
   int    *blk_row = nullptr;
   int     nslice = 0;
   int    *sl_off = nullptr;
   int    *sl_meta = nullptr;
   int    *sl_col = nullptr;
   double *sl_val = nullptr;
   const int *offd_rowptr = nullptr;
   bool    sl_offd_flags = false;
   bool    coarse_op = false;
   bool    owns = true;
};

int  csr_alloc(DevCSR &A, int nrows, int ncols, int nnz, bool values = true);
void csr_free(DevCSR &A);
int  csr_analyze(DevCSR &A);
int  tune_set(const char *key, double value);
bool tune_amg_keep_debug();
int64_t tune_replicate_rows();
int64_t tune_graph_rows();

enum SpmvMode
{
   SPMV_SET = 0,
   SPMV_RESIDUAL = 1,
   SPMV_JACOBI = 2,
   SPMV_ADD = 3,
   SPMV_AXPBY = 4,
   SPMV_JACOBI_R = 5,
   SPMV_SET_DIV = 6,
   SPMV_JACOBI2 = 7,
   SPMV_GS_STEP = 8
};

enum FinOp
{
   FIN_NONE = 0,
   FIN_STORE = 1,
   FIN_SDOTP = 2,
   FIN_IPROD = 3,
   FIN_GAMMA = 4
};

enum ScalIdx
{
   S_BIPROD = 0, S_GAMMA = 1, S_GAMMA_OLD = 2, S_SDOTP = 3, S_IPROD = 4, S_ALPHA = 5, S_BETA = 6,
   S_TMP0 = 8, S_TMP1 = 9, S_TMP2 = 10, S_TMP3 = 11, S_H0 = 16
};

}
struct hdk_csr_s;
namespace hdk {
struct SpmvArgs
{
   const double *x = nullptr;
   double       *y = nullptr;
   const double *b = nullptr;
   const double *d = nullptr;
   const double *xo = nullptr;
   double       *y2 = nullptr;
   double        w = 1.0, alpha = 1.0, beta = 0.0;
   const double *dotv = nullptr;
   int           fin = FIN_NONE;
   double       *fin_out = nullptr;
   const struct ::hdk_csr_s *export_to = nullptr;
   bool          export_y2 = false;
};


int vec_fill(double *x, double v, int64_t n);
int vec_copy(double *dst, const double *src, int64_t n);
int vec_axpy(double a, const double *x, double *y, int64_t n);
int vec_scale(double a, double *x, int64_t n);
int vec_dot_dev(const double *x, const double *y, int64_t n, int fin, double *out_d);
int vec_dot_host(const double *x, const double *y, int64_t n, double *out_h);
int vec_scaled_div(double *u, const double *f, const double *d, double w, int64_t n,
                   const struct ::hdk_csr_s *export_to = nullptr);
int pcg_update_xr(double *x, double *r, const double *p, const double *s, int64_t n, double *scal,
                  int fin = FIN_IPROD, double *fin_out = nullptr,
                  double *z0 = nullptr, const double *zd = nullptr, double zw = 1.0,
                  const struct ::hdk_csr_s *export_z0_to = nullptr);
int pcg_update_p(double *p, const double *z, int64_t n, const double *scal, const struct ::hdk_csr_s *export_to = nullptr);
int vec_copy_dot(double *z, const double *r, int64_t n, int fin, double *out_d);
int allreduce_dev(double *buf_d, int count);
int allreduce_fin_dev(double *buf_d, int count, int fin, double *fin_out);

constexpr int IPC_MAXP = 8;
struct IpcSendArgs
{
   double             *dst[IPC_MAXP];
   int                 off[IPC_MAXP + 1];
   int                 npeer;
   unsigned long long *flag[IPC_MAXP];
   const unsigned long long *rflag;
   int                 nflag;
   unsigned long long  seq;
   unsigned           *ticket;
};
struct HaloExport
{
   const int          *dir = nullptr, *ptr = nullptr, *slot = nullptr;
   int                 total = 0;
   int                 lo_end = 0, hi_begin = 0;
   double             *dst[IPC_MAXP];
   int                 off[IPC_MAXP + 1];
   int                 npeer = 0;
   unsigned long long *flag[IPC_MAXP];
   const unsigned long long *rflag = nullptr;
   int                 nflag = 0;
   unsigned long long  seq = 0;
   unsigned           *ticket = nullptr;
};

struct OffdFuse
{
   const int    *orp = nullptr, *ocol = nullptr;
   const double *oval = nullptr, *xh = nullptr;
};
int spmv_launch(const DevCSR &A, int mode, const SpmvArgs &a, const OffdFuse *of = nullptr);

struct IpcHalo
{
   bool                on = false;
   int64_t             region_off = -1;
   size_t              region_bytes = 0;
   double             *xh[2] = {nullptr, nullptr};
   unsigned long long *data_flag = nullptr;
   double             *dst[2][IPC_MAXP];
   unsigned long long *nbr_flag[IPC_MAXP];
   int                 nnbr = 0;
   unsigned long long  seq = 0;
   unsigned           *tickets = nullptr;
   int                *exp_dir = nullptr, *exp_ptr = nullptr, *exp_slot = nullptr;
   int                 exp_lo_end = 0, exp_hi_begin = 0;
   bool                preposted = false;
};

#ifdef __CUDACC__
__device__ __forceinline__ unsigned long long ld_acquire_sys_u64(const unsigned long long *p)
{
   unsigned long long v;
   asm volatile("ld.acquire.sys.global.u64 %0, [%1];" : "=l"(v) : "l"(p) : "memory");
   return v;
}
__device__ __forceinline__ void st_release_sys_u64(unsigned long long *p, unsigned long long v)
{
   asm volatile("st.release.sys.global.u64 [%0], %1;" ::"l"(p), "l"(v) : "memory");
}
static __device__ long long d_wait_tmo = 0;
static __device__ int      *d_wait_err = nullptr;
static __device__ __noinline__ void wait_seq_slow(const unsigned long long *p, unsigned long long want)
{
   const long long t0 = clock64(), tmo = d_wait_tmo;
   int            *err = d_wait_err;
   unsigned        spins = 0;
   while (ld_acquire_sys_u64(p) < want)
   {
      __nanosleep(64);
      if (tmo > 0 && (++spins & 1023u) == 0)
      {
         if (clock64() - t0 > tmo) { if (err) *(volatile int *)err = 1; return; }
         if (err && *(volatile int *)err) return;
      }
   }
}
__device__ __forceinline__ void wait_seq_sys(const unsigned long long *p, unsigned long long want, long long = 0, int * = nullptr)
{
   if (ld_acquire_sys_u64(p) >= want) return;
   wait_seq_slow(p, want);
}
static inline cudaError_t wait_globals_set(long long tmo, int *err)
{
   cudaError_t e = cudaMemcpyToSymbol(d_wait_tmo, &tmo, sizeof(tmo));
   if (e == cudaSuccess) e = cudaMemcpyToSymbol(d_wait_err, &err, sizeof(err));
   return e;
}
__device__ __forceinline__ int export_row(const HaloExport &e, int r, double v)
{
   if (e.seq == 0 || (r >= e.lo_end && r < e.hi_begin)) return 0;
   const int i = e.dir[r < e.lo_end ? r : e.lo_end + (r - e.hi_begin)];
   if (i < 0) return 0;
   const int k0 = e.ptr[i], k1 = e.ptr[i + 1];
   for (int k = k0; k < k1; k++)
   {
      const int s = e.slot[k];
      int       p = 0;
      while (p + 1 < e.npeer && s >= e.off[p + 1]) p++;
      e.dst[p][s - e.off[p]] = v;
   }
   return k1 - k0;
}
__device__ __forceinline__ void exchange_complete(unsigned long long *const *flag, const unsigned long long *rflag, int nflag,
                                                  unsigned long long seq)
{
   __threadfence_system();
   for (int p = 0; p < nflag; p++) st_release_sys_u64(flag[p], seq);
   for (int p = 0; p < nflag; p++) wait_seq_sys(rflag + p, seq);
}
__device__ __forceinline__ void export_finish(const HaloExport &e, int cnt)
{
   if (e.seq == 0) return;
   const unsigned tot = __reduce_add_sync(0xffffffffu, (unsigned)cnt);
   __syncwarp();
   if (tot == 0 || (threadIdx.x & 31) != 0) return;
   __threadfence_system();
   const unsigned before = atomicAdd(e.ticket, tot);
   if (before + tot == (unsigned)e.total)
   {
      *e.ticket = 0u;
      exchange_complete(e.flag, e.rflag, e.nflag, e.seq);
   }
}
#endif

struct IpcGather
{
   bool                on = false;
   int64_t             n = 0, region_off = -1;
   size_t              region_bytes = 0;
   unsigned long long  seq = 0;
   unsigned long long *flags = nullptr;
   double             *buf[2] = {nullptr, nullptr};
   double             *peer_buf[2][16];
   unsigned long long *peer_flag[16];
   unsigned           *ticket = nullptr;
};
int     ipc_gather_alloc(IpcGather &G, int64_t n);
void    ipc_gather_free(IpcGather &G);
double *ipc_gather_buffer(IpcGather &G);
int     ipc_gather(IpcGather &G, int64_t off, int64_t cnt);

struct HaloPlan
{
   IpcHalo             ipc;
   int                 n_halo = 0;
   int64_t            *col_map = nullptr;
   std::vector<int>     recv_rank, recv_off, recv_cnt;
   std::vector<int>     send_rank, send_off, send_cnt;
   int                 n_send = 0;
   int                *send_idx = nullptr;
   double             *send_buf = nullptr;
   double             *x_halo = nullptr;
};

}

struct hdk_csr_s
{
   int64_t       row_start = 0, row_end = -1, global_rows = 0, global_nnz = 0;
   int64_t       col_start = 0, col_end = -1, global_cols = 0;
   int64_t      *orig_indptr = nullptr, *orig_cols = nullptr;
   double       *orig_vals = nullptr;
   int64_t       orig_nnz = 0;
   int          *offd_rows = nullptr;
   int           n_offd_rows = 0;
   hdk::DevCSR   diag, offd;
   hdk::HaloPlan halo;
   std::vector<int64_t> row_starts;
};

namespace hdk {
int parcsr_matvec(const hdk_csr_s &A, int mode, SpmvArgs a);
bool parcsr_single_kernel(const hdk_csr_s &A);
int parcsr_build(int64_t rs, int64_t re, int64_t cs, int64_t ce, int64_t grows, int64_t gcols, bool square,
                 bool distributed, bool keep_orig, const int64_t *indptr, const int64_t *cols, const double *vals,
                 hdk_csr_s **out, bool analyze = true);
int allreduce_max_dev(double *buf_d, int count);
int bcast_bytes(void *buf_d, size_t bytes, int root);
int allgather_i64_host(int64_t mine, std::vector<int64_t> &all);
int allgather_i32_host(const int *mine, int cnt, std::vector<int> &all);
int allreduce_i32_dev(int *buf_d, int count);
int alltoallv_bytes(const void *send_d, const int64_t *soff , void *recv_d, const int64_t *roff );
int allgatherv_bytes(void *base_d, const int64_t *byte_offs );
void halo_plan_free(HaloPlan &H);
const double *halo_buffer(const hdk_csr_s &A);
int halo_exchange_begin(const hdk_csr_s &A, const double *x);
void dbg_skip_exchange(bool on);
void tl_mark(int level, int op);
int halo_exchange_end(const hdk_csr_s &A);
bool halo_export_begin(const hdk_csr_s &A, HaloExport *e);
void halo_export_cancel(const hdk_csr_s &A);
int comm_check_error();
int wait_globals_spmv(long long tmo, int *err);
int wait_globals_csr(long long tmo, int *err);
int wait_globals_vec(long long tmo, int *err);

__device__ __forceinline__ double warp_sum(double v)
{
#pragma unroll
   for (int o = 16; o > 0; o >>= 1) v += __shfl_down_sync(0xffffffffu, v, o);
   return v;
}

template <int THREADS>
__device__ __forceinline__ double block_sum(double v, double *sm )
{
   int lane = threadIdx.x & 31, w = threadIdx.x >> 5;
   v = warp_sum(v);
   if (lane == 0) sm[w] = v;
   __syncthreads();
   double r = 0.0;
   if (w == 0)
   {
      r = (lane < THREADS / 32) ? sm[lane] : 0.0;
      r = warp_sum(r);
   }
   return r;
}

__device__ __forceinline__ void apply_fin(int fin, double v, double *out, double *scal)
{
   switch (fin)
   {
      case FIN_STORE: out[0] = v; break;
      case FIN_SDOTP: scal[S_SDOTP] = v; scal[S_ALPHA] = (v != 0.0) ? scal[S_GAMMA] / v : 0.0; break;
      case FIN_IPROD: scal[S_IPROD] = v; break;
      case FIN_GAMMA:
      {
         double go = scal[S_GAMMA];
         scal[S_GAMMA_OLD] = go; scal[S_GAMMA] = v; scal[S_BETA] = v / go;
         break;
      }
      default: break;
   }
}

template <int THREADS>
__device__ __forceinline__ void grid_finish(double blocksum, double *partials, unsigned *ticket,
                                            int fin, double *out, double *scal, double *sm,
                                            int *flag_sm)
{
   if (threadIdx.x == 0)
   {
      partials[blockIdx.x] = blocksum;
      __threadfence();
      unsigned t = atomicInc(ticket, gridDim.x - 1);
      *flag_sm   = (t == gridDim.x - 1);
   }
   __syncthreads();
   if (*flag_sm)
   {
      __threadfence();
      double s = 0.0;
      for (unsigned i = threadIdx.x; i < gridDim.x; i += THREADS) s += __ldcg(partials + i);
      __syncthreads();
      s = block_sum<THREADS>(s, sm);
      if (threadIdx.x == 0) apply_fin(fin, s, out, scal);
   }
}

}
```

### hypredrive_b200/csrc/hdk_spmv.cu

```cuda
#include "hdk_internal.cuh"
#include "hdk_amg.cuh"
#include <stdlib.h>
#include <string.h>
#include <map>

namespace hdk {

constexpr int ST       = 256;
constexpr int S_TGT_LO = 1024;
constexpr int S_TGT_HI = 8192;
constexpr int S_MAXR   = 1024;

struct Tune
{
   double rows_mult     = 1.0;
   double tgt_max       = 3072;
   double lpr           = 0;
   double sell_min_rows = 200000;
   double sell_min_rows_dist = 30000;
   double sell_min_avg  = 0.0;
   double sell_sort     = 1;
   double amg_keep_debug = 0;
   double replicate_rows = 262144;
   double export_max_rows = 1e18;
   double graph_rows    = 150000;
   bool   env_read      = false;
};
static Tune tune;
static const struct { const char *key, *env; double Tune::*field; } tune_keys[] = {
   {"spmv_rows_mult", "HDK_SPMV_ROWS_MULT", &Tune::rows_mult}, {"spmv_tgt_max", "HDK_SPMV_TGT_MAX", &Tune::tgt_max},
   {"spmv_lpr", "HDK_SPMV_LPR", &Tune::lpr},                   {"sell_min_rows", "HDK_SELL_MIN_ROWS", &Tune::sell_min_rows},
   {"sell_min_rows_dist", "HDK_SELL_MIN_ROWS_DIST", &Tune::sell_min_rows_dist},
   {"amg_keep_debug", "HDK_AMG_KEEP_DEBUG", &Tune::amg_keep_debug},
   {"replicate_rows", "HDK_REPLICATE_ROWS", &Tune::replicate_rows},
   {"graph_rows", "HDK_GRAPH_ROWS", &Tune::graph_rows},
   {"export_max_rows", "HDK_EXPORT_MAX_ROWS", &Tune::export_max_rows},
   {"sell_min_avg", "HDK_SELL_MIN_AVG", &Tune::sell_min_avg},  {"sell_sort", "HDK_SELL_SORT", &Tune::sell_sort}};
static Tune &tunables()
{
   if (!tune.env_read)
   {
      tune.env_read = true;
      for (const auto &k : tune_keys)
      {
         const char *e = getenv(k.env);
         if (e && *e) tune.*(k.field) = atof(e);
      }
   }
   return tune;
}
bool tune_amg_keep_debug() { return tunables().amg_keep_debug != 0.0; }
int64_t tune_replicate_rows() { return (int64_t)tunables().replicate_rows; }
int64_t tune_graph_rows() { return (int64_t)tunables().graph_rows; }

int tune_set(const char *key, double value)
{
   Tune &t = tunables();
   for (const auto &k : tune_keys)
      if (!strcmp(key, k.key)) { t.*(k.field) = value; return HDK_OK; }
   return set_error(HDK_ERR_INVALID, "unknown tunable '%s'", key);
}

struct SpmvDev
{
   const int    *rowptr, *col, *blk_row;
   const double *val;
   const double *x, *b, *d, *dotv;
   double       *y, *y2;
   double        w, alpha, beta;
   int           nrows, fin;
   double       *fin_out, *scal, *partials;
   unsigned     *ticket;
   const int    *sl_off, *sl_meta, *sl_col;
   const double *sl_val;
   int           nslice;
   const int    *orp, *ocol;
   const double *oval, *xh;
   int           has_halo;

   HaloExport    exp;
   int           exp_y2;
};

__device__ __forceinline__ uint32_t smem_u32(const void *p) { return (uint32_t)__cvta_generic_to_shared(p); }
__device__ __forceinline__ void mbar_init(uint32_t bar, uint32_t count)
{
   asm volatile("mbarrier.init.shared::cta.b64 [%0], %1;" ::"r"(bar), "r"(count));
}
__device__ __forceinline__ void mbar_expect_tx(uint32_t bar, uint32_t bytes)
{
   asm volatile("mbarrier.arrive.expect_tx.shared::cta.b64 _, [%0], %1;" ::"r"(bar), "r"(bytes) : "memory");
}
__device__ __forceinline__ void tma_load_1d(uint32_t dst, const void *src, uint32_t bytes, uint32_t bar)
{
   asm volatile("cp.async.bulk.shared::cluster.global.mbarrier::complete_tx::bytes [%0], [%1], %2, [%3];"
                ::"r"(dst), "l"(src), "r"(bytes), "r"(bar) : "memory");
}
__device__ __forceinline__ void mbar_wait(uint32_t bar, uint32_t parity)
{
   asm volatile("{\n"
                ".reg .pred P1;\n"
                "LAB_WAIT:\n"
                "mbarrier.try_wait.parity.shared::cta.b64 P1, [%0], %1;\n"
                "@P1 bra DONE;\n"
                "bra LAB_WAIT;\n"
                "DONE:\n"
                "}" ::"r"(bar), "r"(parity) : "memory");
}

template <int MODE, bool EXP = false>
__device__ __forceinline__ double store_out(const SpmvDev &a, int r, double v, double dd, double xo, int &nexp)
{
   double yn = v, y2 = 0.0;
   if (MODE == SPMV_JACOBI2)
   {
      yn = __dadd_rn(xo, v);
      y2 = v;
      a.y2[r] = y2;
   }
   else if (MODE == SPMV_GS_STEP)
   {
      y2 = (dd != 0.0) ? __ddiv_rn(v, dd) : 0.0;
      yn = __dadd_rn(a.y[r], __dmul_rn(a.alpha, y2));
      if (a.y2) a.y2[r] = y2;
   }
   else if (MODE == SPMV_SET_DIV)
   {
      y2 = (dd != 0.0) ? __ddiv_rn(__dmul_rn(a.w, v), dd) : 0.0;
      a.y2[r] = y2;
   }
   a.y[r] = yn;
   if (EXP && a.exp.seq) nexp += export_row(a.exp, r, a.exp_y2 ? y2 : yn);
   return yn;
}

template <int MODE>
__device__ __forceinline__ double store_out(const SpmvDev &a, int r, double v, double dd, double xo)
{
   int none = 0;
   return store_out<MODE, false>(a, r, v, dd, xo, none);
}

struct BlkMeta { int r0, r1, k0, k1; };
__device__ __forceinline__ BlkMeta blk_meta(const SpmvDev &a, int b)
{
   BlkMeta m;
   m.r0 = __ldg(a.blk_row + b);
   m.r1 = __ldg(a.blk_row + b + 1);
   m.k0 = __ldg(a.rowptr + m.r0);
   m.k1 = __ldg(a.rowptr + m.r1);
   return m;
}

struct RowOps
{
   int    s, e;
   double b, d, xo, yo, dv;
};

template <int MODE, bool DOT>
__device__ __forceinline__ void row_load(const SpmvDev &a, int r, int ka, RowOps &o)
{
   o.s = __ldg(a.rowptr + r) - ka;
   o.e = __ldg(a.rowptr + r + 1) - ka;
   if (MODE == SPMV_RESIDUAL || MODE == SPMV_JACOBI || MODE == SPMV_JACOBI_R || MODE == SPMV_JACOBI2) o.b = a.b[r];
   if (MODE == SPMV_JACOBI || MODE == SPMV_JACOBI_R || MODE == SPMV_SET_DIV || MODE == SPMV_JACOBI2 || MODE == SPMV_GS_STEP) o.d = a.d[r];
   if (MODE == SPMV_JACOBI || MODE == SPMV_JACOBI2) o.xo = a.x[r];
   if (MODE == SPMV_ADD || MODE == SPMV_AXPBY) o.yo = a.y[r];
   if (DOT) o.dv = a.dotv[r];
}

template <int MODE>
__device__ __forceinline__ double row_compute(const SpmvDev &a, const RowOps &o, const double *vs, const int *cs)
{
   constexpr bool SUB = (MODE == SPMV_RESIDUAL || MODE == SPMV_JACOBI || MODE == SPMV_JACOBI_R || MODE == SPMV_JACOBI2);
   double acc = SUB ? o.b : ((MODE == SPMV_ADD) ? o.yo : 0.0);
   int    k = o.s;
   for (; k + 4 <= o.e; k += 4)
   {
      int    c0 = cs[k], c1 = cs[k + 1], c2 = cs[k + 2], c3 = cs[k + 3];
      double x0 = __ldg(a.x + c0), x1 = __ldg(a.x + c1), x2 = __ldg(a.x + c2), x3 = __ldg(a.x + c3);
      double p0 = __dmul_rn(vs[k], x0), p1 = __dmul_rn(vs[k + 1], x1);
      double p2 = __dmul_rn(vs[k + 2], x2), p3 = __dmul_rn(vs[k + 3], x3);
      if (SUB) { acc = __dadd_rn(acc, -p0); acc = __dadd_rn(acc, -p1); acc = __dadd_rn(acc, -p2); acc = __dadd_rn(acc, -p3); }
      else { acc = __dadd_rn(acc, p0); acc = __dadd_rn(acc, p1); acc = __dadd_rn(acc, p2); acc = __dadd_rn(acc, p3); }
   }
   if (k < o.e)
   {
      int    c0 = cs[k], c1 = (k + 1 < o.e) ? cs[k + 1] : c0, c2 = (k + 2 < o.e) ? cs[k + 2] : c0;
      double x0 = __ldg(a.x + c0), x1 = __ldg(a.x + c1), x2 = __ldg(a.x + c2);
      double p0 = __dmul_rn(vs[k], x0);
      acc       = __dadd_rn(acc, SUB ? -p0 : p0);
      if (k + 1 < o.e) { double p1 = __dmul_rn(vs[k + 1], x1); acc = __dadd_rn(acc, SUB ? -p1 : p1); }
      if (k + 2 < o.e) { double p2 = __dmul_rn(vs[k + 2], x2); acc = __dadd_rn(acc, SUB ? -p2 : p2); }
   }
   if (MODE == SPMV_SET || MODE == SPMV_SET_DIV || MODE == SPMV_ADD || MODE == SPMV_RESIDUAL || MODE == SPMV_GS_STEP) return acc;
   if (MODE == SPMV_AXPBY)
      return (a.beta == 0.0) ? __dmul_rn(a.alpha, acc) : __dadd_rn(__dmul_rn(a.alpha, acc), __dmul_rn(a.beta, o.yo));
   if (MODE == SPMV_JACOBI)
      return (o.d != 0.0) ? __dadd_rn(o.xo, __ddiv_rn(__dmul_rn(a.w, acc), o.d)) : o.xo;
   return (o.d != 0.0) ? __ddiv_rn(__dmul_rn(a.w, acc), o.d) : 0.0;
}

template <int LPR>
__device__ __forceinline__ double row_partial(const SpmvDev &a, int k, int e, const double *vs, const int *cs)
{
   double acc = 0.0;
   for (; k + 3 * LPR < e; k += 4 * LPR)
   {
      int    c0 = cs[k], c1 = cs[k + LPR], c2 = cs[k + 2 * LPR], c3 = cs[k + 3 * LPR];
      double x0 = __ldg(a.x + c0), x1 = __ldg(a.x + c1), x2 = __ldg(a.x + c2), x3 = __ldg(a.x + c3);
      acc = __dadd_rn(acc, __dmul_rn(vs[k], x0));
      acc = __dadd_rn(acc, __dmul_rn(vs[k + LPR], x1));
      acc = __dadd_rn(acc, __dmul_rn(vs[k + 2 * LPR], x2));
      acc = __dadd_rn(acc, __dmul_rn(vs[k + 3 * LPR], x3));
   }
   for (; k < e; k += LPR) acc = __dadd_rn(acc, __dmul_rn(vs[k], __ldg(a.x + cs[k])));
   return acc;
}

template <int MODE>
__device__ __forceinline__ double row_finish(const SpmvDev &a, const RowOps &o, double total)
{
   if (MODE == SPMV_SET || MODE == SPMV_SET_DIV || MODE == SPMV_GS_STEP) return total;
   if (MODE == SPMV_ADD) return __dadd_rn(o.yo, total);
   if (MODE == SPMV_AXPBY)
      return (a.beta == 0.0) ? __dmul_rn(a.alpha, total) : __dadd_rn(__dmul_rn(a.alpha, total), __dmul_rn(a.beta, o.yo));
   double res = __dadd_rn(o.b, -total);
   if (MODE == SPMV_RESIDUAL) return res;
   if (MODE == SPMV_JACOBI)
      return (o.d != 0.0) ? __dadd_rn(o.xo, __ddiv_rn(__dmul_rn(a.w, res), o.d)) : o.xo;
   return (o.d != 0.0) ? __ddiv_rn(__dmul_rn(a.w, res), o.d) : 0.0;
}

template <int MODE, bool DOT, int LPR>
__global__ void __launch_bounds__(ST, 4) k_spmv_tma(SpmvDev a, int nblk, int cap)
{
   constexpr int PF  = 2;
   constexpr int RPB = ST / LPR;
   extern __shared__ __align__(128) unsigned char smem_raw[];
   __shared__ double red[ST / 32];
   __shared__ int    flag;
   double *vbuf = reinterpret_cast<double *>(smem_raw + 128);
   int    *cbuf = reinterpret_cast<int *>(smem_raw + 128 + (size_t)2 * cap * sizeof(double));
   const uint32_t bar0 = smem_u32(smem_raw), bar1 = bar0 + 8;
   const int tid = threadIdx.x, G = gridDim.x;
   if (tid == 0)
   {
      mbar_init(bar0, 1);
      mbar_init(bar1, 1);
      asm volatile("fence.mbarrier_init.release.cluster;" ::: "memory");
   }
   __syncthreads();
   int      b = blockIdx.x, nb = b + G;
   int      stage = 0;
   uint32_t ph0 = 0u, ph1 = 0u;
   double   dacc = 0.0;
   BlkMeta  cur = BlkMeta{0, 0, 0, 0}, nxt = BlkMeta{0, 0, 0, 0};
   if (b < nblk)
   {
      cur = blk_meta(a, b);
      int ka = cur.k0 & ~3, len4 = (cur.k1 - ka + 3) & ~3;
      if (tid == 0 && len4 > 0)
      {
         mbar_expect_tx(bar0, (uint32_t)len4 * 12u);
         tma_load_1d(smem_u32(vbuf), a.val + ka, (uint32_t)len4 * 8u, bar0);
         tma_load_1d(smem_u32(cbuf), a.col + ka, (uint32_t)len4 * 4u, bar0);
      }
   }
   if (nb < nblk) nxt = blk_meta(a, nb);
   while (b < nblk)
   {
      if (nb < nblk && tid == 0)
      {
         int ka = nxt.k0 & ~3, len4 = (nxt.k1 - ka + 3) & ~3;
         if (len4 > 0)
         {
            const uint32_t bar = stage ? bar0 : bar1;
            asm volatile("fence.proxy.async.shared::cta;" ::: "memory");
            mbar_expect_tx(bar, (uint32_t)len4 * 12u);
            tma_load_1d(smem_u32(vbuf + (size_t)(stage ^ 1) * cap), a.val + ka, (uint32_t)len4 * 8u, bar);
            tma_load_1d(smem_u32(cbuf + (size_t)(stage ^ 1) * cap), a.col + ka, (uint32_t)len4 * 4u, bar);
         }
      }
      const int nnb = nb + G;
      BlkMeta   nn  = BlkMeta{0, 0, 0, 0};
      if (nnb < nblk) nn = blk_meta(a, nnb);
      const int ka = cur.k0 & ~3, len = cur.k1 - ka;
      RowOps    ro[PF];
#pragma unroll
      for (int j = 0; j < PF; ++j)
      {
         int r = cur.r0 + tid / LPR + j * RPB;
         if (r < cur.r1) row_load<MODE, DOT>(a, r, ka, ro[j]);
      }
      const double *vs = vbuf + (size_t)stage * cap;
      const int    *cs = cbuf + (size_t)stage * cap;
      if (len > 0)
      {
         if (stage) { mbar_wait(bar1, ph1); ph1 ^= 1u; }
         else { mbar_wait(bar0, ph0); ph0 ^= 1u; }
      }
      if (LPR == 1)
      {
#pragma unroll
         for (int j = 0; j < PF; ++j)
         {
            int r = cur.r0 + tid + j * ST;
            if (r < cur.r1)
            {
               double yn = store_out<MODE>(a, r, row_compute<MODE>(a, ro[j], vs, cs), ro[j].d, ro[j].xo);
               if (DOT) dacc += ro[j].dv * yn;
            }
         }
         for (int r = cur.r0 + tid + PF * ST; r < cur.r1; r += ST)
         {
            RowOps o;
            row_load<MODE, DOT>(a, r, ka, o);
            double yn = store_out<MODE>(a, r, row_compute<MODE>(a, o, vs, cs), o.d, o.xo);
            if (DOT) dacc += o.dv * yn;
         }
      }
      else
      {
         const int sub = tid % LPR, rl = tid / LPR;
#pragma unroll
         for (int j = 0; j < PF; ++j)
         {
            int    r = cur.r0 + rl + j * RPB;
            bool   valid = r < cur.r1;
            double part = valid ? row_partial<LPR>(a, ro[j].s + sub, ro[j].e, vs, cs) : 0.0;
#pragma unroll
            for (int o = LPR / 2; o > 0; o >>= 1) part = __dadd_rn(part, __shfl_xor_sync(0xffffffffu, part, o));
            if (valid && sub == 0)
            {
               double yn = store_out<MODE>(a, r, row_finish<MODE>(a, ro[j], part), ro[j].d, ro[j].xo);
               if (DOT) dacc += ro[j].dv * yn;
            }
         }
         for (int base = cur.r0 + PF * RPB; base < cur.r1; base += RPB)
         {
            int    r = base + rl;
            bool   valid = r < cur.r1;
            RowOps o;
            o.s = o.e = 0;
            if (valid) row_load<MODE, DOT>(a, r, ka, o);
            double part = valid ? row_partial<LPR>(a, o.s + sub, o.e, vs, cs) : 0.0;
#pragma unroll
            for (int w = LPR / 2; w > 0; w >>= 1) part = __dadd_rn(part, __shfl_xor_sync(0xffffffffu, part, w));
            if (valid && sub == 0)
            {
               double yn = store_out<MODE>(a, r, row_finish<MODE>(a, o, part), o.d, o.xo);
               if (DOT) dacc += o.dv * yn;
            }
         }
      }
      __syncthreads();
      b = nb; nb = nnb; cur = nxt; nxt = nn; stage ^= 1;
   }
   if (DOT)
   {
      double bs = block_sum<ST>(dacc, red);
      __syncthreads();
      grid_finish<ST>(bs, a.partials, a.ticket, a.fin, a.fin_out, a.scal, red, &flag);
   }
}

constexpr int SELL_T = 256;
constexpr int SELL_OFFD_BIT = 32;

template <int MODE>
__device__ __forceinline__ double row_epilogue(const SpmvDev &a, const RowOps &o, double acc)
{
   if (MODE == SPMV_SET || MODE == SPMV_SET_DIV || MODE == SPMV_ADD || MODE == SPMV_RESIDUAL || MODE == SPMV_GS_STEP) return acc;
   if (MODE == SPMV_AXPBY)
      return (a.beta == 0.0) ? __dmul_rn(a.alpha, acc) : __dadd_rn(__dmul_rn(a.alpha, acc), __dmul_rn(a.beta, o.yo));
   if (MODE == SPMV_JACOBI)
      return (o.d != 0.0) ? __dadd_rn(o.xo, __ddiv_rn(__dmul_rn(a.w, acc), o.d)) : o.xo;
   return (o.d != 0.0) ? __ddiv_rn(__dmul_rn(a.w, acc), o.d) : 0.0;
}

#ifdef HDK_XHINT
__device__ __forceinline__ uint64_t x_policy()
{
   uint64_t pol;
   asm volatile("createpolicy.fractional.L2::evict_last.b64 %0, 1.0;" : "=l"(pol));
   return pol;
}
__device__ __forceinline__ double ld_x(const double *p, uint64_t pol)
{
   double v;
   asm volatile("ld.global.nc.L2::cache_hint.f64 %0, [%1], %2;" : "=d"(v) : "l"(p), "l"(pol));
   return v;
}
#define LDX(p) ld_x((p), xpol)
#else
#define LDX(p) __ldg(p)
#endif
template <int MODE, bool DOT, bool OFFD, bool EXP>
__device__ __forceinline__ void sell_body(const SpmvDev &a)
{
#ifdef HDK_XHINT
   const uint64_t xpol = x_policy();
#endif
   constexpr bool SUB  = (MODE == SPMV_RESIDUAL || MODE == SPMV_JACOBI || MODE == SPMV_JACOBI_R || MODE == SPMV_JACOBI2);
   constexpr bool DIAG = (MODE == SPMV_JACOBI || MODE == SPMV_JACOBI_R || MODE == SPMV_SET_DIV || MODE == SPMV_JACOBI2 || MODE == SPMV_GS_STEP);
   constexpr bool XOLD = (MODE == SPMV_JACOBI || MODE == SPMV_JACOBI2);
   __shared__ double red[SELL_T / 32];
   __shared__ int    flag;
   const int lane = threadIdx.x & 31;
   const int wpb  = SELL_T / 32;
   __shared__ double s_dot[DOT ? SELL_T : 1];
   if (DOT) s_dot[threadIdx.x] = 0.0;
   int nexp = 0;
   for (int s = blockIdx.x * wpb + (threadIdx.x >> 5); s < a.nslice; s += gridDim.x * wpb)
   {
      const int  meta  = __ldg(a.sl_meta + (size_t)s * 32 + lane);
      const int  len   = meta >> 6;
      const int  r     = s * 32 + (meta & 31);
      const bool valid = r < a.nrows;
      const size_t base = (size_t)__ldg(a.sl_off + s) * 32 + lane;
      RowOps o;
      o.b = o.d = o.xo = o.yo = o.dv = 0.0;
      constexpr bool LATE = DOT;
      if (valid)
      {
         if (SUB) o.b = a.b[r];
         if (!LATE && DIAG) o.d = a.d[r];
         if (!LATE && XOLD) o.xo = a.x[r];
         if (MODE == SPMV_AXPBY) o.yo = a.y[r];
      }
      double        acc = SUB ? o.b : 0.0;
      const int    *cp  = a.sl_col + base;
      const double *vp  = a.sl_val + base;
      int    c0 = 0, c1 = 0, c2 = 0, c3 = 0;
      double v0 = 0.0, v1 = 0.0, v2 = 0.0, v3 = 0.0;
      if (0 < len) { c0 = __ldcs(cp); v0 = __ldcs(vp); }
      if (1 < len) { c1 = __ldcs(cp + 32); v1 = __ldcs(vp + 32); }
      if (2 < len) { c2 = __ldcs(cp + 64); v2 = __ldcs(vp + 64); }
      if (3 < len) { c3 = __ldcs(cp + 96); v3 = __ldcs(vp + 96); }
#pragma unroll 1
      for (int k = 0; k < len; k += 4)
      {
         const double x0 = LDX(a.x + c0), x1 = LDX(a.x + c1), x2 = LDX(a.x + c2), x3 = LDX(a.x + c3);
         const size_t q  = (size_t)(k + 4) * 32;
         int          n0 = 0, n1 = 0, n2 = 0, n3 = 0;
         double       w0 = 0.0, w1 = 0.0, w2 = 0.0, w3 = 0.0;
         if (k + 4 < len) { n0 = __ldcs(cp + q); w0 = __ldcs(vp + q); }
         if (k + 5 < len) { n1 = __ldcs(cp + q + 32); w1 = __ldcs(vp + q + 32); }
         if (k + 6 < len) { n2 = __ldcs(cp + q + 64); w2 = __ldcs(vp + q + 64); }
         if (k + 7 < len) { n3 = __ldcs(cp + q + 96); w3 = __ldcs(vp + q + 96); }
         const double p0 = __dmul_rn(v0, x0), p1 = __dmul_rn(v1, x1), p2 = __dmul_rn(v2, x2), p3 = __dmul_rn(v3, x3);
         acc = __dadd_rn(acc, SUB ? -p0 : p0);
         if (k + 1 < len) acc = __dadd_rn(acc, SUB ? -p1 : p1);
         if (k + 2 < len) acc = __dadd_rn(acc, SUB ? -p2 : p2);
         if (k + 3 < len) acc = __dadd_rn(acc, SUB ? -p3 : p3);
         c0 = n0; c1 = n1; c2 = n2; c3 = n3;
         v0 = w0; v1 = w1; v2 = w2; v3 = w3;
      }
      if (OFFD && (meta & SELL_OFFD_BIT))
      {
         for (int k = __ldg(a.orp + r), e = __ldg(a.orp + r + 1); k < e; ++k)
         {
            const double p0 = __dmul_rn(__ldg(a.oval + k), __ldcg(a.xh + __ldg(a.ocol + k)));
            acc = __dadd_rn(acc, SUB ? -p0 : p0);
         }
      }
      if (valid)
      {
         if (LATE && DIAG) o.d = a.d[r];
         if (LATE && XOLD) o.xo = a.x[r];
         if (DOT) o.dv = a.dotv[r];
         if (MODE == SPMV_ADD) acc = __dadd_rn(a.y[r], acc);
         double yn = store_out<MODE, EXP>(a, r, row_epilogue<MODE>(a, o, acc), o.d, o.xo, nexp);
         if (DOT) s_dot[threadIdx.x] += o.dv * yn;
      }
   }
   if (EXP) export_finish(a.exp, nexp);
   if (DOT)
   {
      double bs = block_sum<SELL_T>(s_dot[threadIdx.x], red);
      __syncthreads();
      grid_finish<SELL_T>(bs, a.partials, a.ticket, a.fin, a.fin_out, a.scal, red, &flag);
   }
}

template <int MODE, bool DOT, bool OFFD, bool EXP>
__global__ void __launch_bounds__(SELL_T) k_spmv_sell(SpmvDev a) { sell_body<MODE, DOT, OFFD, EXP>(a); }

__global__ void k_sell_meta(const int *rowptr, int nrows, int nslice, int *meta, int *width, int *max_slice_nnz,
                            const int *offd_rowptr)
{
   const int lane = threadIdx.x & 31;
   const int s    = blockIdx.x * (blockDim.x >> 5) + (threadIdx.x >> 5);
   if (s >= nslice) return;
   const int r   = s * 32 + lane;
   const int len = (r < nrows) ? rowptr[r + 1] - rowptr[r] : 0;
   const int key = (r < nrows) ? len : -1;
   int       rank = 0, w = 0;
   for (int j = 0; j < 32; ++j)
   {
      int kj = __shfl_sync(0xffffffffu, key, j);
      rank += (kj > key) || (kj == key && j < lane);
      w = kj > w ? kj : w;
   }
   const int ob = (offd_rowptr && r < nrows && offd_rowptr[r + 1] > offd_rowptr[r]) ? SELL_OFFD_BIT : 0;
   meta[(size_t)s * 32 + rank] = (len << 6) | lane | ob;
   if (lane == 0)
   {
      width[s] = w;
      int hi   = s * 32 + 32;
      if (hi > nrows) hi = nrows;
      atomicMax(max_slice_nnz, rowptr[hi] - rowptr[s * 32]);
   }
}

template <bool SORT>
__global__ void k_sell_fill(const int *rowptr, const int *col, const double *val, int nrows, int nslice, const int *sl_off,
                            const int *meta, int *scol, double *sval, int cap)
{
   extern __shared__ __align__(16) unsigned char sm_raw[];
   const int lane = threadIdx.x & 31, w = threadIdx.x >> 5, nw = blockDim.x >> 5;
   double   *vs = reinterpret_cast<double *>(sm_raw) + (size_t)w * cap;
   int      *cs = reinterpret_cast<int *>(sm_raw + (size_t)nw * cap * sizeof(double)) + (size_t)w * cap;
   const int s  = blockIdx.x * nw + w;
   if (s >= nslice) return;
   int hi = s * 32 + 32;
   if (hi > nrows) hi = nrows;
   const int k0 = rowptr[s * 32], k1 = rowptr[hi];
   for (int k = k0 + lane; k < k1; k += 32) { cs[k - k0] = col[k]; vs[k - k0] = val[k]; }
   __syncwarp();
   const int m = meta[(size_t)s * 32 + lane], len = m >> 6, r = s * 32 + (m & 31);
   if (r >= nrows || len == 0) return;
   const int rs = rowptr[r] - k0;
   if (SORT)
   {
      const int b = rs + ((cs[rs] == r) ? 1 : 0), e = rs + len;
      for (int k = b + 1; k < e; ++k)
      {
         int    c = cs[k];
         double v = vs[k];
         int    j = k - 1;
         while (j >= b && cs[j] > c) { cs[j + 1] = cs[j]; vs[j + 1] = vs[j]; --j; }
         cs[j + 1] = c; vs[j + 1] = v;
      }
   }
   const size_t base = (size_t)sl_off[s] * 32 + lane;
   for (int k = 0; k < len; ++k)
   {
      scol[base + (size_t)k * 32] = cs[rs + k];
      sval[base + (size_t)k * 32] = vs[rs + k];
   }
}

template <int MODE, bool DOT, bool OFFD, bool EXP>
static int launch_sell_v(const DevCSR &A, const SpmvDev &d)
{
   static int occ = 0;
   if (!occ)
   {
      HDK_CUDA(cudaOccupancyMaxActiveBlocksPerMultiprocessor(&occ, k_spmv_sell<MODE, DOT, OFFD, EXP>, SELL_T, 0));
      if (occ < 1) occ = 1;
   }
   int grid = cdiv(A.nslice, SELL_T / 32);
   int cap  = g.sm_count * occ;
   if (grid > cap) grid = cap;
   k_spmv_sell<MODE, DOT, OFFD, EXP><<<grid, SELL_T, 0, g.stream>>>(d);
   return HDK_OK;
}
template <int MODE, bool DOT>
static int launch_sell(const DevCSR &A, const SpmvDev &d)
{
   if (!d.has_halo) return launch_sell_v<MODE, DOT, false, false>(A, d);
   return d.exp.seq ? launch_sell_v<MODE, DOT, true, true>(A, d) : launch_sell_v<MODE, DOT, true, false>(A, d);
}

template <int MODE, bool DOT>
__global__ void __launch_bounds__(ST) k_spmv_vector(SpmvDev a)
{
   __shared__ double red[ST / 32];
   __shared__ int    flag;
   const int lane = threadIdx.x & 31;
   const int wpb  = ST / 32;
   double    dacc = 0.0;
   for (int r = blockIdx.x * wpb + (threadIdx.x >> 5); r < a.nrows; r += gridDim.x * wpb)
   {
      int    s = a.rowptr[r], e = a.rowptr[r + 1];
      double acc = 0.0;
      for (int k = s + lane; k < e; k += 32) acc += __ldg(a.val + k) * __ldg(a.x + __ldg(a.col + k));
      acc = warp_sum(acc);
      if (lane == 0)
      {
         double yn;
         if (MODE == SPMV_SET || MODE == SPMV_SET_DIV || MODE == SPMV_GS_STEP) yn = acc;
         else if (MODE == SPMV_AXPBY) yn = (a.beta == 0.0) ? a.alpha * acc : a.alpha * acc + a.beta * a.y[r];
         else if (MODE == SPMV_ADD) yn = a.y[r] + acc;
         else
         {
            double res = a.b[r] - acc;
            if (MODE == SPMV_RESIDUAL) yn = res;
            else
            {
               double dd = a.d[r];
               if (MODE == SPMV_JACOBI) yn = (dd != 0.0) ? a.x[r] + (a.w * res) / dd : a.x[r];
               else yn = (dd != 0.0) ? (a.w * res) / dd : 0.0;
            }
         }
         constexpr bool NEED_D = (MODE == SPMV_SET_DIV || MODE == SPMV_GS_STEP);
         yn = store_out<MODE>(a, r, yn, NEED_D ? a.d[r] : 0.0, MODE == SPMV_JACOBI2 ? a.x[r] : 0.0);
         if (DOT) dacc += a.dotv[r] * yn;
      }
   }
   if (DOT)
   {
      double bs = block_sum<ST>(dacc, red);
      __syncthreads();
      grid_finish<ST>(bs, a.partials, a.ticket, a.fin, a.fin_out, a.scal, red, &flag);
   }
}

template <int MODE, bool DOT, int LPR>
static int launch_tma(const DevCSR &A, const SpmvDev &d)
{
   static bool                  attr_set = false;
   static std::map<size_t, int> occ_cache;
   size_t                       smem = 128 + (size_t)2 * A.cap * 12;
   if (!attr_set)
   {
      HDK_CUDA(cudaFuncSetAttribute(k_spmv_tma<MODE, DOT, LPR>, cudaFuncAttributeMaxDynamicSharedMemorySize, 226 * 1024));
      attr_set = true;
   }
   auto it = occ_cache.find(smem);
   if (it == occ_cache.end())
   {
      int occ = 0;
      HDK_CUDA(cudaOccupancyMaxActiveBlocksPerMultiprocessor(&occ, k_spmv_tma<MODE, DOT, LPR>, ST, smem));
      if (occ < 1) occ = 1;
      it = occ_cache.emplace(smem, occ).first;
   }
   int grid = g.sm_count * it->second;
   if (grid > A.nblk) grid = A.nblk;
   k_spmv_tma<MODE, DOT, LPR><<<grid, ST, smem, g.stream>>>(d, A.nblk, A.cap);
   return HDK_OK;
}

template <int MODE>
static int launch_mode(const DevCSR &A, const SpmvDev &d, bool dot)
{
   if (A.kind == 0)
   {
      switch (A.lpr)
      {
         case 2: if (dot) HDK_TRY((launch_tma<MODE, true, 2>(A, d))); else HDK_TRY((launch_tma<MODE, false, 2>(A, d))); break;
         case 4: if (dot) HDK_TRY((launch_tma<MODE, true, 4>(A, d))); else HDK_TRY((launch_tma<MODE, false, 4>(A, d))); break;
         case 8: if (dot) HDK_TRY((launch_tma<MODE, true, 8>(A, d))); else HDK_TRY((launch_tma<MODE, false, 8>(A, d))); break;
         default: if (dot) HDK_TRY((launch_tma<MODE, true, 1>(A, d))); else HDK_TRY((launch_tma<MODE, false, 1>(A, d))); break;
      }
   }
   else if (A.kind == 2)
   {
      if (dot) HDK_TRY((launch_sell<MODE, true>(A, d))); else HDK_TRY((launch_sell<MODE, false>(A, d)));
   }
   else
   {
      int grid = cdiv(A.nrows, ST / 32);
      int cap  = g.sm_count * 16;
      if (grid > cap) grid = cap;
      if (grid < 1) grid = 1;
      if (dot) k_spmv_vector<MODE, true><<<grid, ST, 0, g.stream>>>(d);
      else k_spmv_vector<MODE, false><<<grid, ST, 0, g.stream>>>(d);
   }
   HDK_LAUNCH_CHECK();
   return HDK_OK;
}

int spmv_launch(const DevCSR &A, int mode, const SpmvArgs &s, const OffdFuse *of)
{
   if (A.nrows <= 0) return HDK_OK;
   SpmvDev d;
   d.rowptr = A.rowptr; d.col = A.col; d.val = A.val; d.blk_row = A.blk_row;
   d.x = s.x; d.b = s.b; d.d = s.d; d.dotv = s.dotv; d.y = s.y; d.y2 = s.y2;
   d.w = s.w; d.alpha = s.alpha; d.beta = s.beta;
   d.nrows = A.nrows; d.fin = s.fin; d.fin_out = s.fin_out;
   d.scal = g.dscal; d.partials = g.partials; d.ticket = g.counters;
   d.sl_off = A.sl_off; d.sl_meta = A.sl_meta; d.sl_col = A.sl_col; d.sl_val = A.sl_val; d.nslice = A.nslice;
   d.orp = nullptr; d.ocol = nullptr; d.oval = nullptr; d.xh = nullptr; d.has_halo = 0;
   if (of)
   {
      if (A.kind != 2 || !A.sl_offd_flags) return set_error(HDK_ERR_INVALID, "fused off-rank block needs the sliced-ELL layout with flagged rows");
      d.orp = of->orp; d.ocol = of->ocol; d.oval = of->oval; d.xh = of->xh;
      d.has_halo = 1;
   }
   d.exp = HaloExport();
   d.exp_y2 = s.export_y2 ? 1 : 0;
   if (s.export_to && of && (double)A.nrows <= tunables().export_max_rows) halo_export_begin(*s.export_to, &d.exp);
   bool dot = (s.fin != FIN_NONE && s.dotv != nullptr);
   switch (mode)
   {
      case SPMV_SET: return launch_mode<SPMV_SET>(A, d, dot);
      case SPMV_RESIDUAL: return launch_mode<SPMV_RESIDUAL>(A, d, dot);
      case SPMV_JACOBI: return launch_mode<SPMV_JACOBI>(A, d, dot);
      case SPMV_ADD: return launch_mode<SPMV_ADD>(A, d, dot);
      case SPMV_AXPBY: return launch_mode<SPMV_AXPBY>(A, d, dot);
      case SPMV_JACOBI_R: return launch_mode<SPMV_JACOBI_R>(A, d, dot);
      case SPMV_SET_DIV: return launch_mode<SPMV_SET_DIV>(A, d, dot);
      case SPMV_JACOBI2: return launch_mode<SPMV_JACOBI2>(A, d, dot);
      case SPMV_GS_STEP: return launch_mode<SPMV_GS_STEP>(A, d, dot);
   }
   return set_error(HDK_ERR_INVALID, "unknown spmv mode %d", mode);
}

__global__ void k_row_stats(const int *rowptr, int nrows, int *max_row)
{
   int m = 0;
   for (int r = blockIdx.x * blockDim.x + threadIdx.x; r < nrows; r += gridDim.x * blockDim.x)
   {
      int l = rowptr[r + 1] - rowptr[r];
      m     = l > m ? l : m;
   }
   for (int o = 16; o > 0; o >>= 1) { int t = __shfl_down_sync(0xffffffffu, m, o); m = t > m ? t : m; }
   if ((threadIdx.x & 31) == 0 && m > 0) atomicMax(max_row, m);
}

__global__ void k_blk_rows(const int *rowptr, int nrows, int nblk, int tgt, int *blk_row)
{
   int b = blockIdx.x * blockDim.x + threadIdx.x;
   if (b > nblk) return;
   if (b == nblk) { blk_row[b] = nrows; return; }
   int target = b * tgt;
   int lo = 0, hi = nrows;
   while (lo < hi)
   {
      int mid = (lo + hi) >> 1;
      if (rowptr[mid] >= target) hi = mid; else lo = mid + 1;
   }
   blk_row[b] = lo;
}

static void sell_free(DevCSR &A)
{
   dfree(A.sl_off); dfree(A.sl_meta); dfree(A.sl_col); dfree(A.sl_val);
   A.sl_off = A.sl_meta = A.sl_col = nullptr; A.sl_val = nullptr; A.nslice = 0;
}

static int sell_build(DevCSR &A)
{
   const bool sort = tunables().sell_sort != 0.0 && A.coarse_op;
   const int ns = cdiv(A.nrows, 32);
   int      *width = nullptr, *dmax = reinterpret_cast<int *>(g.dscal + S_TMP3);
   HDK_TRY(dalloc(&A.sl_meta, (size_t)ns * 32));
   HDK_TRY(dalloc(&A.sl_off, (size_t)ns + 1));
   HDK_TRY(dalloc(&width, (size_t)ns + 1));
   HDK_CUDA(cudaMemsetAsync(width + ns, 0, sizeof(int), g.stream));
   HDK_CUDA(cudaMemsetAsync(dmax, 0, sizeof(int), g.stream));
   static int fuse_on = -1;
   if (fuse_on < 0) { const char *e = getenv("HDK_FUSE_OFFD"); fuse_on = (e && atoi(e) == 0) ? 0 : 1; }
   const int *orp = fuse_on ? A.offd_rowptr : nullptr;
   k_sell_meta<<<cdiv(ns, 8), 256, 0, g.stream>>>(A.rowptr, A.nrows, ns, A.sl_meta, width, dmax, orp);
   A.sl_offd_flags = (orp != nullptr);
   HDK_LAUNCH_CHECK();
   HDK_TRY(exclusive_scan_int(width, A.sl_off, ns + 1));
   int h[2] = {0, 0};
   HDK_CUDA(cudaMemcpyAsync(&h[0], A.sl_off + ns, sizeof(int), cudaMemcpyDeviceToHost, g.stream));
   HDK_CUDA(cudaMemcpyAsync(&h[1], dmax, sizeof(int), cudaMemcpyDeviceToHost, g.stream));
   HDK_CUDA(cudaStreamSynchronize(g.stream));
   dfree(width);
   const int64_t padded = (int64_t)h[0] * 32;
   const int     cap    = (h[1] + 3) & ~3;
   int           nw     = 4;
   while (nw > 1 && (size_t)nw * cap * 12 > 200 * 1024) nw >>= 1;
   if (padded > 3 * (int64_t)A.nnz + 4096 || (size_t)nw * cap * 12 > 200 * 1024) { sell_free(A); return HDK_OK; }
   HDK_TRY(dalloc(&A.sl_col, (size_t)padded + 32));
   HDK_TRY(dalloc(&A.sl_val, (size_t)padded + 32));
   const size_t smem = (size_t)nw * cap * 12;
   const bool   do_sort = sort && A.nrows == A.ncols;
   if (do_sort)
   {
      HDK_CUDA(cudaFuncSetAttribute(k_sell_fill<true>, cudaFuncAttributeMaxDynamicSharedMemorySize, 200 * 1024));
      k_sell_fill<true><<<cdiv(ns, nw), nw * 32, smem, g.stream>>>(A.rowptr, A.col, A.val, A.nrows, ns, A.sl_off, A.sl_meta,
                                                                    A.sl_col, A.sl_val, cap);
   }
   else
   {
      HDK_CUDA(cudaFuncSetAttribute(k_sell_fill<false>, cudaFuncAttributeMaxDynamicSharedMemorySize, 200 * 1024));
      k_sell_fill<false><<<cdiv(ns, nw), nw * 32, smem, g.stream>>>(A.rowptr, A.col, A.val, A.nrows, ns, A.sl_off, A.sl_meta,
                                                                     A.sl_col, A.sl_val, cap);
   }
   HDK_LAUNCH_CHECK();
   A.nslice = ns;
   A.kind   = 2;
   return HDK_OK;
}

int csr_analyze(DevCSR &A)
{
   if (A.blk_row) { dfree(A.blk_row); A.blk_row = nullptr; }
   sell_free(A);
   A.nblk = 0; A.kind = 0; A.max_row = 0; A.avg_row = 0.0;
   if (A.nrows <= 0) return HDK_OK;
   int *dmax = reinterpret_cast<int *>(g.dscal + S_TMP3);
   HDK_CUDA(cudaMemsetAsync(dmax, 0, sizeof(int), g.stream));
   int grid = cdiv(A.nrows, 256);
   if (grid > g.sm_count * 8) grid = g.sm_count * 8;
   k_row_stats<<<grid, 256, 0, g.stream>>>(A.rowptr, A.nrows, dmax);
   HDK_LAUNCH_CHECK();
   int hmax = 0;
   HDK_CUDA(cudaMemcpyAsync(&hmax, dmax, sizeof(int), cudaMemcpyDeviceToHost, g.stream));
   HDK_CUDA(cudaStreamSynchronize(g.stream));
   A.max_row = hmax;
   A.avg_row = (double)A.nnz / (double)A.nrows;
   A.kind    = (hmax <= S_MAXR) ? 0 : 1;
   if (A.kind == 0 && A.val)
   {
      const Tune &t = tunables();
      const double min_rows = A.offd_rowptr ? t.sell_min_rows_dist : t.sell_min_rows;
      if ((double)A.nrows >= min_rows && A.avg_row > t.sell_min_avg) HDK_TRY(sell_build(A));
   }
   if (A.kind == 0)
   {
      const Tune &t = tunables();
      double mult = t.rows_mult > 0 ? t.rows_mult : 1.0;
      int    thi  = (int)t.tgt_max;
      if (thi < S_TGT_LO) thi = S_TGT_LO;
      if (thi > S_TGT_HI) thi = S_TGT_HI;
      const int lpr_force = (int)t.lpr;
      int lpr = A.avg_row <= 12.0 ? 1 : (A.avg_row <= 24.0 ? 2 : (A.avg_row <= 56.0 ? 4 : 8));
      if (lpr_force == 1 || lpr_force == 2 || lpr_force == 4 || lpr_force == 8) lpr = lpr_force;
      A.lpr   = lpr;
      int tgt = ((int)(A.avg_row * (256.0 / lpr) * mult) / 64) * 64;
      if (tgt < S_TGT_LO) tgt = S_TGT_LO;
      if (tgt > thi) tgt = thi;
      A.tgt  = tgt;
      A.cap  = (tgt + hmax + 8 + 3) & ~3;
      A.nblk = A.nnz / tgt + 1;
      if (A.nblk > PARTIALS_CAP) return set_error(HDK_ERR_UNSUPPORTED, "matrix too large for the reduction scratch");
      HDK_TRY(dalloc(&A.blk_row, (size_t)A.nblk + 1));
      k_blk_rows<<<cdiv(A.nblk + 1, 256), 256, 0, g.stream>>>(A.rowptr, A.nrows, A.nblk, tgt, A.blk_row);
      HDK_LAUNCH_CHECK();
   }
   return HDK_OK;
}

int csr_alloc(DevCSR &A, int nrows, int ncols, int nnz, bool values)
{
   A.nrows = nrows; A.ncols = ncols; A.nnz = nnz; A.owns = true;
   HDK_TRY(dalloc(&A.rowptr, (size_t)nrows + 1));
   HDK_TRY(dalloc(&A.col, (size_t)nnz + 8));
   HDK_CUDA(cudaMemsetAsync(A.col + nnz, 0, sizeof(int) * 8, g.stream));
   if (values)
   {
      HDK_TRY(dalloc(&A.val, (size_t)nnz + 8));
      HDK_CUDA(cudaMemsetAsync(A.val + nnz, 0, sizeof(double) * 8, g.stream));
   }
   else A.val = nullptr;
   return HDK_OK;
}

void csr_free(DevCSR &A)
{
   if (A.owns) { dfree(A.rowptr); dfree(A.col); dfree(A.val); }
   dfree(A.blk_row);
   sell_free(A);
   A = DevCSR();
}

int wait_globals_spmv(long long tmo, int *err)
{
   return wait_globals_set(tmo, err) == cudaSuccess ? HDK_OK : set_error(HDK_ERR_CUDA, "cannot set the wait budget");
}

}
```

### hypredrive_b200/hdk.py

```python
from __future__ import annotations

import ctypes as C
import os

import numpy as np

_HERE = os.path.dirname(os.path.abspath(__file__))
LIB_PATH = os.environ.get("HDK_LIB") or os.path.join(_HERE, "lib", "libHYPREDRV.so")
_lib = None


class HdkError(RuntimeError):
    pass


class AmgParams(C.Structure):
    _fields_ = [("coarsen_type", C.c_int), ("strong_th", C.c_double), ("max_row_sum", C.c_double),
                ("max_coarse_size", C.c_int), ("min_coarse_size", C.c_int), ("max_levels", C.c_int),
                ("interp_type", C.c_int), ("max_nnz_row", C.c_int), ("trunc_factor", C.c_double),
                ("relax_down", C.c_int), ("relax_up", C.c_int), ("relax_coarse", C.c_int),
                ("sweeps_down", C.c_int), ("sweeps_up", C.c_int), ("sweeps_coarse", C.c_int),
                ("relax_weight", C.c_double), ("outer_weight", C.c_double), ("rand_seed", C.c_int),
                ("keep_transpose", C.c_int), ("print_level", C.c_int)]


class Krylov(C.Structure):
    _fields_ = [("max_iter", C.c_int), ("rel_tol", C.c_double), ("abs_tol", C.c_double),
                ("krylov_dim", C.c_int), ("min_iter", C.c_int), ("skip_real_res_check", C.c_int),
                ("iters", C.c_int), ("converged", C.c_int), ("rel_res_norm", C.c_double),
                ("solve_ms", C.c_double)]


def lib():
    global _lib
    if _lib is None:
        if not os.path.exists(LIB_PATH):
            raise HdkError(f"{LIB_PATH} is missing: run `python -c 'import __graft_entry__ as g; g.build()'` "
                           "(nvcc, sm_100a). hypredrive_b200 has no CPU fallback.")
        L = C.CDLL(LIB_PATH, mode=C.RTLD_GLOBAL)
        L.hdk_last_error.restype = C.c_char_p
        L.hdk_stream.restype = C.c_void_p
        L.hdk_launch_count_reset.restype = C.c_int64
        L.hdk_amg_operator_complexity.restype = C.c_double
        L.hdk_amg_operator_complexity.argtypes = [C.c_void_p]
        L.hdk_amg_vcycle_bytes.restype = C.c_double
        L.hdk_amg_vcycle_bytes.argtypes = [C.c_void_p]
        L.hdk_amg_num_levels.argtypes = [C.c_void_p]
        L.hdk_vec_fill.argtypes = [C.c_void_p, C.c_double, C.c_int64]
        L.hdk_vec_axpy.argtypes = [C.c_double, C.c_void_p, C.c_void_p, C.c_int64]
        L.hdk_vec_scale.argtypes = [C.c_double, C.c_void_p, C.c_int64]
        L.hdk_vec_alloc.argtypes = [C.c_int64, C.POINTER(C.c_void_p)]
        L.hdk_vec_free.argtypes = [C.c_void_p]
        L.hdk_vec_h2d.argtypes = [C.c_void_p, C.c_void_p, C.c_int64]
        L.hdk_vec_d2h.argtypes = [C.c_void_p, C.c_void_p, C.c_int64]
        L.hdk_vec_copy.argtypes = [C.c_void_p, C.c_void_p, C.c_int64]
        L.hdk_vec_dot.argtypes = [C.c_void_p, C.c_void_p, C.c_int64, C.POINTER(C.c_double)]
        L.hdk_vec_norm.argtypes = [C.c_void_p, C.c_int64, C.c_int, C.POINTER(C.c_double)]
        L.hdk_vec_random.argtypes = [C.c_void_p, C.c_int64, C.c_int64, C.c_int]
        L.hdk_csr_from_host.argtypes = [C.c_int64, C.c_int64, C.c_int64, C.c_void_p, C.c_void_p, C.c_void_p,
                                        C.POINTER(C.c_void_p)]
        L.hdk_csr_stencil.argtypes = [C.c_int, C.c_int, C.c_int, C.c_int, C.POINTER(C.c_double), C.c_int64,
                                      C.c_int64, C.POINTER(C.c_void_p), C.c_void_p]
        L.hdk_csr_destroy.argtypes = [C.c_void_p]
        L.hdk_csr_info.argtypes = [C.c_void_p] + [C.POINTER(C.c_int64)] * 4
        L.hdk_csr_get_diag.argtypes = [C.c_void_p, C.c_void_p, C.c_void_p, C.c_void_p]
        L.hdk_csr_matvec.argtypes = [C.c_void_p, C.c_double, C.c_void_p, C.c_double, C.c_void_p]
        L.hdk_csr_residual.argtypes = [C.c_void_p, C.c_void_p, C.c_void_p, C.c_void_p]
        L.hdk_csr_spmv_kind.argtypes = [C.c_void_p, C.POINTER(C.c_int), C.POINTER(C.c_double), C.POINTER(C.c_int)]
        L.hdk_amg_default_params.argtypes = [C.POINTER(AmgParams)]
        L.hdk_amg_setup.argtypes = [C.c_void_p, C.POINTER(AmgParams), C.POINTER(C.c_void_p)]
        L.hdk_amg_destroy.argtypes = [C.c_void_p]
        L.hdk_amg_apply.argtypes = [C.c_void_p, C.c_void_p, C.c_void_p]
        L.hdk_amg_vcycle.argtypes = [C.c_void_p, C.c_void_p, C.c_void_p]
        L.hdk_amg_level_info.argtypes = [C.c_void_p, C.c_int] + [C.POINTER(C.c_int64)] * 3
        L.hdk_amg_get_matrix.argtypes = [C.c_void_p, C.c_int, C.c_int, C.c_void_p, C.c_void_p, C.c_void_p]
        L.hdk_amg_get_cf.argtypes = [C.c_void_p, C.c_int, C.c_void_p]
        L.hdk_amg_get_measure.argtypes = [C.c_void_p, C.c_int, C.c_void_p]
        L.hdk_amg_get_l1.argtypes = [C.c_void_p, C.c_int, C.c_void_p]
        L.hdk_pcg.argtypes = [C.c_void_p, C.c_void_p, C.c_void_p, C.c_void_p, C.POINTER(Krylov)]
        L.hdk_gmres.argtypes = [C.c_void_p, C.c_void_p, C.c_void_p, C.c_void_p, C.POINTER(Krylov)]
        L.hdk_fgmres.argtypes = [C.c_void_p, C.c_void_p, C.c_void_p, C.c_void_p, C.POINTER(Krylov)]
        L.hdk_bicgstab.argtypes = [C.c_void_p, C.c_void_p, C.c_void_p, C.c_void_p, C.POINTER(Krylov)]
        L.hdk_time_kernel.argtypes = [C.c_void_p, C.c_void_p, C.c_int, C.c_int, C.POINTER(C.c_double),
                                      C.POINTER(C.c_double)]
        L.hdk_comm_unique_id.argtypes = [C.c_void_p]
        L.hdk_comm_init.argtypes = [C.c_int, C.c_int, C.c_void_p]
        L.hdk_init.argtypes = [C.c_int]
        _lib = L
    return _lib


def check(rc: int):
    if rc != 0:
        raise HdkError(f"hdk error {rc}: {lib().hdk_last_error().decode(errors='replace')}")


def init(device: int = -1):
    check(lib().hdk_init(device))


def device_count() -> int:
    return lib().hdk_device_count()


class DVec:

    def __init__(self, n: int, data: np.ndarray | None = None):
        self.n = int(n)
        self.p = C.c_void_p()
        check(lib().hdk_vec_alloc(self.n, C.byref(self.p)))
        if data is not None:
            self.set(data)

    def set(self, data):
        a = np.ascontiguousarray(data, dtype=np.float64)
        assert a.size == self.n
        check(lib().hdk_vec_h2d(self.p, a.ctypes.data, self.n))

    def get(self) -> np.ndarray:
        out = np.empty(self.n, dtype=np.float64)
        if self.n:
            check(lib().hdk_vec_d2h(out.ctypes.data, self.p, self.n))
        return out

    def fill(self, v: float):
        check(lib().hdk_vec_fill(self.p, float(v), self.n))

    def free(self):
        if self.p:
            lib().hdk_vec_free(self.p)
            self.p = C.c_void_p()

    def __del__(self):
        try:
            self.free()
        except Exception:
            pass


class DCsr:

    def __init__(self, handle):
        self.h = handle

    @classmethod
    def from_csr(cls, indptr, cols, data, row_start=0, row_end=None, global_rows=None):
        ip = np.ascontiguousarray(indptr, dtype=np.int64)
        cj = np.ascontiguousarray(cols, dtype=np.int64)
        va = np.ascontiguousarray(data, dtype=np.float64)
        n = ip.size - 1
        if row_end is None:
            row_end = row_start + n - 1
        if global_rows is None:
            global_rows = row_end + 1
        h = C.c_void_p()
        check(lib().hdk_csr_from_host(row_start, row_end, global_rows, ip.ctypes.data, cj.ctypes.data,
                                      va.ctypes.data, C.byref(h)))
        return cls(h)

    @classmethod
    def from_scipy(cls, A):
        A = A.tocsr()
        return cls.from_csr(A.indptr, A.indices, A.data)

    @classmethod
    def stencil(cls, kind: int, nx: int, ny: int, nz: int, c=(1.0, 1.0, 1.0), row_start=0, row_end=None):
        n = nx * ny * nz
        if row_end is None:
            row_end = n - 1
        h = C.c_void_p()
        b = DVec(row_end - row_start + 1)
        cc = (C.c_double * 3)(*map(float, c))
        check(lib().hdk_csr_stencil(kind, nx, ny, nz, cc, row_start, row_end, C.byref(h), b.p))
        return cls(h), b

    def info(self):
        v = [C.c_int64() for _ in range(4)]
        check(lib().hdk_csr_info(self.h, *[C.byref(x) for x in v]))
        return dict(local_rows=v[0].value, global_rows=v[1].value, local_nnz=v[2].value, global_nnz=v[3].value)

    def diag_arrays(self):
        i = self.info()
        n, nnz = i["local_rows"], i["local_nnz"]
        rp = np.empty(n + 1, dtype=np.int32)
        cj = np.empty(max(nnz, 1), dtype=np.int32)
        va = np.empty(max(nnz, 1), dtype=np.float64)
        check(lib().hdk_csr_get_diag(self.h, rp.ctypes.data, cj.ctypes.data, va.ctypes.data))
        nn = int(rp[n])
        return rp, cj[:nn], va[:nn]

    def matvec(self, x: DVec, y: DVec, alpha=1.0, beta=0.0):
        check(lib().hdk_csr_matvec(self.h, float(alpha), x.p, float(beta), y.p))

    def residual(self, x: DVec, b: DVec, r: DVec):
        check(lib().hdk_csr_residual(self.h, x.p, b.p, r.p))

    def spmv_kind(self):
        k, a, m = C.c_int(), C.c_double(), C.c_int()
        check(lib().hdk_csr_spmv_kind(self.h, C.byref(k), C.byref(a), C.byref(m)))
        return dict(kind=k.value, avg_row=a.value, max_row=m.value)

    def free(self):
        if self.h:
            lib().hdk_csr_destroy(self.h)
            self.h = C.c_void_p()

    def __del__(self):
        try:
            self.free()
        except Exception:
            pass


def amg_params(**kw) -> AmgParams:
    p = AmgParams()
    lib().hdk_amg_default_params(C.byref(p))
    for k, v in kw.items():
        if not hasattr(p, k):
            raise KeyError(k)
        setattr(p, k, v)
    return p


class DAmg:

    def __init__(self, A: DCsr, params: AmgParams | None = None):
        self.params = params if params is not None else amg_params()
        self.h = C.c_void_p()
        self.A = A
        check(lib().hdk_amg_setup(A.h, C.byref(self.params), C.byref(self.h)))

    @property
    def nlev(self):
        return lib().hdk_amg_num_levels(self.h)

    def level_info(self, l):
        v = [C.c_int64() for _ in range(3)]
        check(lib().hdk_amg_level_info(self.h, l, *[C.byref(x) for x in v]))
        return dict(rows=v[0].value, nnz_A=v[1].value, nnz_P=v[2].value)

    def sizes(self):
        return [(self.level_info(l)["rows"], self.level_info(l)["nnz_A"]) for l in range(self.nlev)]

    def matrix(self, l, which):
        code = {"A": 0, "P": 1, "R": 2, "S": 3}[which]
        info = self.level_info(l)
        if which == "A":
            nrows, nnz = info["rows"], info["nnz_A"]
        elif which == "P":
            nrows, nnz = info["rows"], info["nnz_P"]
        elif which == "R":
            nrows, nnz = self.level_info(l + 1)["rows"], info["nnz_P"]
        else:
            nrows, nnz = info["rows"], info["nnz_A"]
        rp = np.empty(nrows + 1, dtype=np.int32)
        cj = np.empty(max(nnz, 1), dtype=np.int32)
        va = np.zeros(max(nnz, 1), dtype=np.float64)
        check(lib().hdk_amg_get_matrix(self.h, l, code, rp.ctypes.data, cj.ctypes.data, va.ctypes.data))
        nn = int(rp[nrows])
        return rp, cj[:nn], va[:nn]

    def cf(self, l):
        out = np.empty(self.level_info(l)["rows"], dtype=np.int32)
        check(lib().hdk_amg_get_cf(self.h, l, out.ctypes.data))
        return out

    def measure(self, l):
        out = np.empty(self.level_info(l)["rows"], dtype=np.float64)
        check(lib().hdk_amg_get_measure(self.h, l, out.ctypes.data))
        return out

    def l1(self, l):
        out = np.empty(self.level_info(l)["rows"], dtype=np.float64)
        check(lib().hdk_amg_get_l1(self.h, l, out.ctypes.data))
        return out

    def apply(self, r: DVec, z: DVec):
        check(lib().hdk_amg_apply(self.h, r.p, z.p))

    def vcycle(self, f: DVec, u: DVec):
        check(lib().hdk_amg_vcycle(self.h, f.p, u.p))

    def operator_complexity(self):
        return lib().hdk_amg_operator_complexity(self.h)

    def vcycle_bytes(self):
        return lib().hdk_amg_vcycle_bytes(self.h)

    def free(self):
        if self.h:
            lib().hdk_amg_destroy(self.h)
            self.h = C.c_void_p()

    def __del__(self):
        try:
            self.free()
        except Exception:
            pass


def pcg(A: DCsr, b: DVec, x: DVec, M: DAmg | None = None, max_iter=100, rel_tol=1e-6, abs_tol=0.0):
    k = Krylov(max_iter=max_iter, rel_tol=rel_tol, abs_tol=abs_tol)
    check(lib().hdk_pcg(A.h, M.h if M is not None else None, b.p, x.p, C.byref(k)))
    return dict(iters=k.iters, converged=bool(k.converged), rel_res_norm=k.rel_res_norm, solve_ms=k.solve_ms)


def gmres(A: DCsr, b: DVec, x: DVec, M: DAmg | None = None, max_iter=300, rel_tol=1e-6, abs_tol=0.0,
          krylov_dim=30, skip_real_res_check=0):
    k = Krylov(max_iter=max_iter, rel_tol=rel_tol, abs_tol=abs_tol, krylov_dim=krylov_dim,
               skip_real_res_check=skip_real_res_check)
    check(lib().hdk_gmres(A.h, M.h if M is not None else None, b.p, x.p, C.byref(k)))
    return dict(iters=k.iters, converged=bool(k.converged), rel_res_norm=k.rel_res_norm, solve_ms=k.solve_ms)


def fgmres(A: DCsr, b: DVec, x: DVec, M: DAmg | None = None, max_iter=300, rel_tol=1e-6, abs_tol=0.0, krylov_dim=30):
    k = Krylov(max_iter=max_iter, rel_tol=rel_tol, abs_tol=abs_tol, krylov_dim=krylov_dim)
    check(lib().hdk_fgmres(A.h, M.h if M is not None else None, b.p, x.p, C.byref(k)))
    return dict(iters=k.iters, converged=bool(k.converged), rel_res_norm=k.rel_res_norm, solve_ms=k.solve_ms)


def bicgstab(A: DCsr, b: DVec, x: DVec, M: DAmg | None = None, max_iter=100, rel_tol=1e-6, abs_tol=0.0):
    k = Krylov(max_iter=max_iter, rel_tol=rel_tol, abs_tol=abs_tol)
    check(lib().hdk_bicgstab(A.h, M.h if M is not None else None, b.p, x.p, C.byref(k)))
    return dict(iters=k.iters, converged=bool(k.converged), rel_res_norm=k.rel_res_norm, solve_ms=k.solve_ms)


def time_kernel(A: DCsr, M: DAmg | None, kernel: int, reps: int = 20):
    ms, by = C.c_double(), C.c_double()
    check(lib().hdk_time_kernel(A.h, M.h if M is not None else None, kernel, reps, C.byref(ms), C.byref(by)))
    return ms.value, by.value


def amg_rows(hM, level: int, which: int):
    L = lib()
    L.hdk_amg_get_rows.argtypes = [C.c_void_p, C.c_int, C.c_int] + [C.POINTER(C.c_int64)] * 3 + [C.c_void_p] * 3
    r0, nr, nz = C.c_int64(), C.c_int64(), C.c_int64()
    check(L.hdk_amg_get_rows(hM, level, which, C.byref(r0), C.byref(nr), C.byref(nz), None, None, None))
    ip = np.empty(nr.value + 1, dtype=np.int64)
    cj = np.empty(max(nz.value, 1), dtype=np.int64)
    va = np.empty(max(nz.value, 1), dtype=np.float64)
    check(L.hdk_amg_get_rows(hM, level, which, None, None, None, ip.ctypes.data, cj.ctypes.data, va.ctypes.data))
    return int(r0.value), ip, cj[:nz.value], va[:nz.value]


def amg_local_levels(hM):
    L = lib()
    L.hdk_amg_num_dist_levels.argtypes = [C.c_void_p]
    return int(L.hdk_amg_num_dist_levels(hM)), int(L.hdk_amg_num_levels(hM))


def tune(key: str, value: float):
    L = lib()
    L.hdk_tune.argtypes = [C.c_char_p, C.c_double]
    check(L.hdk_tune(key.encode(), float(value)))


def launch_count_reset() -> int:
    return int(lib().hdk_launch_count_reset())


def sync():
    check(lib().hdk_sync())
```

### include/hdk.h

```cpp
#ifndef HDK_H
#define HDK_H

#include <stddef.h>
#include <stdint.h>

#ifdef __cplusplus
extern "C" {
#endif

#define HDK_OK 0
#define HDK_ERR_NO_DEVICE 1
#define HDK_ERR_CUDA 2
#define HDK_ERR_INVALID 3
#define HDK_ERR_ALLOC 4
#define HDK_ERR_UNSUPPORTED 5
#define HDK_ERR_COMM 6

typedef struct hdk_csr_s hdk_csr;
typedef struct hdk_amg_s hdk_amg;

int         hdk_init(int device);
int         hdk_finalize(void);
int         hdk_device_count(void);
const char *hdk_last_error(void);
int         hdk_sync(void);
void       *hdk_stream(void);

int hdk_comm_unique_id(void *id128_h);
int hdk_comm_init(int rank, int nranks, const void *id128_h);
int hdk_comm_init_from_env(void);
int hdk_comm_halo_mode(void);
int hdk_comm_rank(void);
int hdk_comm_size(void);
int hdk_comm_finalize(void);
int hdk_comm_max_i64(int64_t local, int64_t *global);
int hdk_comm_sum_i64(int64_t local, int64_t *global);

int hdk_vec_alloc(int64_t n, double **x_d);
int hdk_vec_free(double *x_d);
int hdk_host_alloc(size_t bytes, void **p_h);
int hdk_host_free(void *p_h);
int hdk_vec_h2d(double *x_d, const double *x_h, int64_t n);
int hdk_vec_d2h(double *x_h, const double *x_d, int64_t n);
int hdk_vec_fill(double *x_d, double value, int64_t n);
int hdk_vec_copy(double *dst_d, const double *src_d, int64_t n);
int hdk_vec_axpy(double alpha, const double *x_d, double *y_d, int64_t n);
int hdk_vec_scale(double alpha, double *x_d, int64_t n);
int hdk_vec_dot(const double *x_d, const double *y_d, int64_t n, double *result_h);
int hdk_vec_norm(const double *x_d, int64_t n, int kind, double *result_h);
int hdk_vec_random(double *x_d, int64_t n, int64_t global_offset, int seed);

int hdk_csr_from_host(int64_t row_start, int64_t row_end, int64_t global_rows,
                      const int64_t *indptr_h, const int64_t *cols_h, const double *vals_h,
                      hdk_csr **A);
int hdk_csr_from_device(int64_t row_start, int64_t row_end, int64_t global_rows,
                        const int64_t *indptr_d, const int64_t *cols_d, const double *vals_d,
                        hdk_csr **A);
int hdk_csr_destroy(hdk_csr *A);
int hdk_csr_info(const hdk_csr *A, int64_t *local_rows, int64_t *global_rows,
                 int64_t *local_nnz, int64_t *global_nnz);
int hdk_csr_get_diag(const hdk_csr *A, int32_t *rowptr_h, int32_t *col_h, double *val_h);

int hdk_csr_matvec(const hdk_csr *A, double alpha, const double *x_d, double beta, double *y_d);
int hdk_csr_residual(const hdk_csr *A, const double *x_d, const double *b_d, double *r_d);
int hdk_csr_spmv_kind(const hdk_csr *A, int *kind, double *avg_row, int *max_row);

int hdk_csr_stencil(int kind, int nx, int ny, int nz, const double c[3], int64_t row_start,
                    int64_t row_end, hdk_csr **A, double *b_d);

typedef struct
{
   int    coarsen_type;
   double strong_th;
   double max_row_sum;
   int    max_coarse_size;
   int    min_coarse_size;
   int    max_levels;
   int    interp_type;
   int    max_nnz_row;
   double trunc_factor;
   int    relax_down, relax_up, relax_coarse;
   int    sweeps_down, sweeps_up, sweeps_coarse;
   double relax_weight, outer_weight;
   int    rand_seed;
   int    keep_transpose;
   int    print_level;
} hdk_amg_params;

void hdk_amg_default_params(hdk_amg_params *p);
int  hdk_amg_setup(const hdk_csr *A, const hdk_amg_params *p, hdk_amg **M);
int  hdk_amg_destroy(hdk_amg *M);
int  hdk_amg_apply(hdk_amg *M, const double *r_d, double *z_d);
int  hdk_amg_vcycle(hdk_amg *M, const double *f_d, double *u_d);

int hdk_amg_num_levels(const hdk_amg *M);
int hdk_amg_num_dist_levels(const hdk_amg *M);
int hdk_amg_level_info(const hdk_amg *M, int level, int64_t *rows, int64_t *nnz_A, int64_t *nnz_P);
int hdk_amg_get_matrix(const hdk_amg *M, int level, int which, int32_t *rowptr_h,
                       int32_t *col_h, double *val_h);
int hdk_amg_get_rows(const hdk_amg *M, int level, int which, int64_t *row0, int64_t *nrows, int64_t *nnz,
                     int64_t *indptr_h, int64_t *cols_h, double *vals_h);
int hdk_amg_get_cf(const hdk_amg *M, int level, int32_t *cf_h);
int hdk_amg_get_measure(const hdk_amg *M, int level, double *measure_h);
int hdk_amg_get_l1(const hdk_amg *M, int level, double *l1_h);
double hdk_amg_operator_complexity(const hdk_amg *M);
double hdk_amg_vcycle_bytes(const hdk_amg *M);

int hdk_amg_strength(const hdk_csr *A, double theta, double max_row_sum, int64_t *nnz_S,
                     int32_t **rowptr_d, int32_t **col_d);
int hdk_amg_pmis(int64_t n, const int32_t *S_rowptr_d, const int32_t *S_col_d, int seed,
                 int64_t global_offset, int32_t *cf_d, double *measure_d, int *iterations);
int hdk_free_device(void *p_d);
int hdk_copy_d2h(void *dst_h, const void *src_d, size_t bytes);
int hdk_copy_h2d(void *dst_d, const void *src_h, size_t bytes);
int hdk_malloc_device(void **p_d, size_t bytes);

typedef struct
{
   int    max_iter;
   double rel_tol, abs_tol;
   int    krylov_dim;
   int    min_iter;
   int    skip_real_res_check;
   int    iters, converged;
   double rel_res_norm;
   double solve_ms;
} hdk_krylov;

int hdk_pcg(const hdk_csr *A, hdk_amg *M , const double *b_d, double *x_d,
            hdk_krylov *k);
int hdk_gmres(const hdk_csr *A, hdk_amg *M, const double *b_d, double *x_d, hdk_krylov *k);
int hdk_fgmres(const hdk_csr *A, hdk_amg *M, const double *b_d, double *x_d, hdk_krylov *k);
int hdk_bicgstab(const hdk_csr *A, hdk_amg *M, const double *b_d, double *x_d, hdk_krylov *k);

int hdk_time_kernel(const hdk_csr *A, hdk_amg *M, int kernel, int reps, double *avg_ms,
                    double *algorithmic_bytes);
int64_t hdk_launch_count_reset(void);
int hdk_tune(const char *key, double value);
int hdk_profiler_range(int start);

#ifdef __cplusplus
}
#endif
#endif
```

Before: 5.382 billion.

## Add stencil-compressed SELL slices storing shared relative column offsets per slice

During SELL build, a new classification kernel finds slices whose rows share a common stencil pattern. For those slices it stores a single row of relative column offsets and values, and the SpMV kernel reads them with vectorized int4 loads. This is meant to cut the column and value index traffic that dominates the SpMV on structured Poisson operators. It also moves the diag, x-old and y loads to after the accumulation and adds byte-accounting helpers and a census API. In exchange it widens the meta encoding, adds an extra setup kernel and host sync, and puts a divergent branch in the SpMV body.

Measured after the change: 5.827 billion (median of 6 runs). 1.08x the previous value.

```diff
diff --git a/hypredrive_b200/csrc/hdk_amg_setup.cu b/hypredrive_b200/csrc/hdk_amg_setup.cu
--- a/hypredrive_b200/csrc/hdk_amg_setup.cu
+++ b/hypredrive_b200/csrc/hdk_amg_setup.cu
@@ -1966,15 +1966,15 @@
       bool tsgs = (prm->relax_down == 11 || prm->relax_down == 12 || prm->relax_up == 11 || prm->relax_up == 12);
       if (tsgs && (rc = build_lower(L.A->diag, L.L))) break;
       if (tsgs && ((rc = dalloc(&L.gs1, (size_t)n + 8)) || (rc = dalloc(&L.gs2, (size_t)n + 8)))) break;
-      double nnzA = (double)L.A->diag.nnz + L.A->offd.nnz;
+      const double bA = parcsr_stream_bytes(*L.A);
       if (L.P)
       {
-         double nnzP = (double)L.P->diag.nnz + L.P->offd.nnz, ncl = (double)L.P->diag.ncols;
+         double ncl = (double)L.P->diag.ncols;
          bytes += 24.0 * n;
-         bytes += 12.0 * nnzA + 4.0 * (n + 1) + 24.0 * n;
-         bytes += 12.0 * nnzP + 4.0 * (ncl + 1) + 8.0 * n + 8.0 * ncl;
-         bytes += 12.0 * nnzP + 4.0 * (n + 1) + 16.0 * n + 8.0 * ncl;
-         bytes += 12.0 * nnzA + 4.0 * (n + 1) + 32.0 * n;
+         bytes += bA + 24.0 * n;
+         bytes += parcsr_stream_bytes(*L.R) + 8.0 * n + 8.0 * ncl;
+         bytes += parcsr_stream_bytes(*L.P) + 16.0 * n + 8.0 * ncl;
+         bytes += bA + 32.0 * n;
       }
       else bytes += 8.0 * (double)n * n + 16.0 * n;
    }
@@ -2230,8 +2230,12 @@
       for (int l = tail_level; l < nl; l++)
       {
          AmgLevel &Lg = Mg->lev[(size_t)l];
-         double    n = Lg.n, nnzA = Lg.A->diag.nnz;
-         if (Lg.P) { double nnzP = Lg.P->diag.nnz, ncl = Lg.P->diag.ncols; vb += 24.0 * n + 2 * (12.0 * nnzA + 4.0 * n) + 56.0 * n + 2 * (12.0 * nnzP) + 28.0 * n + 16.0 * ncl; }
+         double    n = Lg.n;
+         if (Lg.P)
+         {
+            double ncl = Lg.P->diag.ncols;
+            vb += 24.0 * n + 2 * csr_stream_bytes(Lg.A->diag) + 56.0 * n + csr_stream_bytes(Lg.R->diag) + csr_stream_bytes(Lg.P->diag) + 28.0 * n + 16.0 * ncl;
+         }
          else vb += 8.0 * n * n + 16.0 * n;
       }
       M->vcycle_bytes = vb;
diff --git a/hypredrive_b200/csrc/hdk_amg_solve.cu b/hypredrive_b200/csrc/hdk_amg_solve.cu
--- a/hypredrive_b200/csrc/hdk_amg_solve.cu
+++ b/hypredrive_b200/csrc/hdk_amg_solve.cu
@@ -385,7 +385,7 @@
    HDK_TRY(require_init());
    if (!A) return set_error(HDK_ERR_INVALID, "null matrix");
    const int64_t n = A->diag.nrows;
-   const double  nnz = (double)A->diag.nnz + A->offd.nnz;
+   const double  ab = parcsr_stream_bytes(*A);
    double *x, *y, *b, *d, *z;
    HDK_TRY(dalloc(&x, (size_t)n + 8)); HDK_TRY(dalloc(&y, (size_t)n + 8));
    HDK_TRY(dalloc(&b, (size_t)n + 8)); HDK_TRY(dalloc(&d, (size_t)n + 8));
@@ -406,9 +406,9 @@
          a.x = x; a.y = y; a.b = b; a.d = d;
          switch (kernel)
          {
-            case 0: rc = parcsr_matvec(*A, SPMV_SET, a); by = 12.0 * nnz + 4.0 * (n + 1) + 16.0 * n; break;
-            case 1: rc = parcsr_matvec(*A, SPMV_JACOBI, a); by = 12.0 * nnz + 4.0 * (n + 1) + 32.0 * n; break;
-            case 2: rc = parcsr_matvec(*A, SPMV_RESIDUAL, a); by = 12.0 * nnz + 4.0 * (n + 1) + 24.0 * n; break;
+            case 0: rc = parcsr_matvec(*A, SPMV_SET, a); by = ab + 16.0 * n; break;
+            case 1: rc = parcsr_matvec(*A, SPMV_JACOBI, a); by = ab + 32.0 * n; break;
+            case 2: rc = parcsr_matvec(*A, SPMV_RESIDUAL, a); by = ab + 24.0 * n; break;
             case 3:
                rc = vec_fill(g.dscal + S_ALPHA, 1e-3, 1);
                if (rc == HDK_OK) rc = pcg_update_xr(y, b, x, d, n, g.dscal, FIN_IPROD, nullptr, z, d, 1.0);
@@ -426,15 +426,15 @@
                else
                {
                   const int    type = (M->prm.relax_down == 12 || M->prm.relax_up == 12) ? 12 : 11;
-                  const double nnzL = (double)M->lev[0].L.nnz;
+                  const double lb   = csr_stream_bytes(M->lev[0].L);
                   rc = relax_sweep(M, 0, type, M->lev[0].l1_down, b, x, y, FIN_NONE, nullptr);
-                  by = 12.0 * nnz + 4.0 * (n + 1) + 40.0 * n + (type == 11 ? 1 : 2) * (12.0 * nnzL + 4.0 * (n + 1) + 32.0 * n) + (type == 12 ? 8.0 * n : 0.0);
+                  by = ab + 40.0 * n + (type == 11 ? 1 : 2) * (lb + 32.0 * n) + (type == 12 ? 8.0 * n : 0.0);
                }
                break;
             case 7: rc = halo_exchange_begin(*A, x); by = 8.0 * A->halo.n_send; break;
             case 8:
                dbg_skip_exchange(true);
-               rc = parcsr_matvec(*A, SPMV_SET, a); by = 12.0 * nnz + 4.0 * (n + 1) + 16.0 * n;
+               rc = parcsr_matvec(*A, SPMV_SET, a); by = ab + 16.0 * n;
                dbg_skip_exchange(false);
                break;
             default: rc = set_error(HDK_ERR_INVALID, "unknown kernel id %d", kernel);
diff --git a/hypredrive_b200/csrc/hdk_csr.cu b/hypredrive_b200/csrc/hdk_csr.cu
--- a/hypredrive_b200/csrc/hdk_csr.cu
+++ b/hypredrive_b200/csrc/hdk_csr.cu
@@ -630,4 +630,13 @@
    return HDK_OK;
 }
 
-}
+int hdk_csr_sell_census(const hdk_csr *A, int64_t *stencil, int64_t *plain, double *bytes)
+{
+   if (!A) return set_error(HDK_ERR_INVALID, "null matrix");
+   if (stencil) *stencil = A->diag.sl_stencil;
+   if (plain) *plain = (int64_t)A->diag.nslice - A->diag.sl_stencil;
+   if (bytes) *bytes = hdk::parcsr_stream_bytes(*A);
+   return HDK_OK;
+}
+
+}
diff --git a/hypredrive_b200/csrc/hdk_internal.cuh b/hypredrive_b200/csrc/hdk_internal.cuh
--- a/hypredrive_b200/csrc/hdk_internal.cuh
+++ b/hypredrive_b200/csrc/hdk_internal.cuh
@@ -93,6 +93,8 @@
    int    *sl_meta = nullptr;
    int    *sl_col = nullptr;
    double *sl_val = nullptr;
+   int     sl_stencil = 0;
+   int64_t sl_stencil_seg = 0, sl_plain_nnz = 0;
    const int *offd_rowptr = nullptr;
    bool    sl_offd_flags = false;
    bool    coarse_op = false;
@@ -102,6 +104,7 @@
 int  csr_alloc(DevCSR &A, int nrows, int ncols, int nnz, bool values = true);
 void csr_free(DevCSR &A);
 int  csr_analyze(DevCSR &A);
+double csr_stream_bytes(const DevCSR &A);
 int  tune_set(const char *key, double value);
 bool tune_amg_keep_debug();
 int64_t tune_replicate_rows();
@@ -348,6 +351,7 @@
 
 namespace hdk {
 int parcsr_matvec(const hdk_csr_s &A, int mode, SpmvArgs a);
+double parcsr_stream_bytes(const hdk_csr_s &A);
 bool parcsr_single_kernel(const hdk_csr_s &A);
 int parcsr_build(int64_t rs, int64_t re, int64_t cs, int64_t ce, int64_t grows, int64_t gcols, bool square,
                  bool distributed, bool keep_orig, const int64_t *indptr, const int64_t *cols, const double *vals,
diff --git a/hypredrive_b200/csrc/hdk_spmv.cu b/hypredrive_b200/csrc/hdk_spmv.cu
--- a/hypredrive_b200/csrc/hdk_spmv.cu
+++ b/hypredrive_b200/csrc/hdk_spmv.cu
@@ -20,6 +20,7 @@
    double sell_min_rows_dist = 30000;
    double sell_min_avg  = 0.0;
    double sell_sort     = 1;
+   double sell_stencil  = 1;
    double amg_keep_debug = 0;
    double replicate_rows = 262144;
    double export_max_rows = 1e18;
@@ -35,7 +36,8 @@
    {"replicate_rows", "HDK_REPLICATE_ROWS", &Tune::replicate_rows},
    {"graph_rows", "HDK_GRAPH_ROWS", &Tune::graph_rows},
    {"export_max_rows", "HDK_EXPORT_MAX_ROWS", &Tune::export_max_rows},
-   {"sell_min_avg", "HDK_SELL_MIN_AVG", &Tune::sell_min_avg},  {"sell_sort", "HDK_SELL_SORT", &Tune::sell_sort}};
+   {"sell_min_avg", "HDK_SELL_MIN_AVG", &Tune::sell_min_avg},  {"sell_sort", "HDK_SELL_SORT", &Tune::sell_sort},
+   {"sell_stencil", "HDK_SELL_STENCIL", &Tune::sell_stencil}};
 static Tune &tunables()
 {
    if (!tune.env_read)
@@ -367,7 +369,9 @@
 }
 
 constexpr int SELL_T = 256;
-constexpr int SELL_OFFD_BIT = 32;
+constexpr int SELL_OFFD_BIT    = 32;
+constexpr int SELL_STENCIL_BIT = 64;
+constexpr int SELL_LEN_SHIFT   = 7;
 
 template <int MODE>
 __device__ __forceinline__ double row_epilogue(const SpmvDev &a, const RowOps &o, double acc)
@@ -415,48 +419,63 @@
    int nexp = 0;
    for (int s = blockIdx.x * wpb + (threadIdx.x >> 5); s < a.nslice; s += gridDim.x * wpb)
    {
-      const int  meta  = __ldg(a.sl_meta + (size_t)s * 32 + lane);
-      const int  len   = meta >> 6;
+      int ln = lane;
+      if (!OFFD) asm volatile("mov.u32 %0, %%laneid;" : "=r"(ln));
+      const int  meta  = __ldg(a.sl_meta + (size_t)s * 32 + ln);
+      const int  len   = meta >> SELL_LEN_SHIFT;
       const int  r     = s * 32 + (meta & 31);
       const bool valid = r < a.nrows;
-      const size_t base = (size_t)__ldg(a.sl_off + s) * 32 + lane;
+      const size_t base = (size_t)__ldg(a.sl_off + s) * 32;
       RowOps o;
       o.b = o.d = o.xo = o.yo = o.dv = 0.0;
-      constexpr bool LATE = DOT;
-      if (valid)
-      {
-         if (SUB) o.b = a.b[r];
-         if (!LATE && DIAG) o.d = a.d[r];
-         if (!LATE && XOLD) o.xo = a.x[r];
-         if (MODE == SPMV_AXPBY) o.yo = a.y[r];
-      }
-      double        acc = SUB ? o.b : 0.0;
-      const int    *cp  = a.sl_col + base;
-      const double *vp  = a.sl_val + base;
-      int    c0 = 0, c1 = 0, c2 = 0, c3 = 0;
-      double v0 = 0.0, v1 = 0.0, v2 = 0.0, v3 = 0.0;
-      if (0 < len) { c0 = __ldcs(cp); v0 = __ldcs(vp); }
-      if (1 < len) { c1 = __ldcs(cp + 32); v1 = __ldcs(vp + 32); }
-      if (2 < len) { c2 = __ldcs(cp + 64); v2 = __ldcs(vp + 64); }
-      if (3 < len) { c3 = __ldcs(cp + 96); v3 = __ldcs(vp + 96); }
+      if (valid && SUB) o.b = a.b[r];
+      double acc = SUB ? o.b : 0.0;
+      if (meta & SELL_STENCIL_BIT)
+      {
 #pragma unroll 1
-      for (int k = 0; k < len; k += 4)
-      {
-         const double x0 = LDX(a.x + c0), x1 = LDX(a.x + c1), x2 = LDX(a.x + c2), x3 = LDX(a.x + c3);
-         const size_t q  = (size_t)(k + 4) * 32;
-         int          n0 = 0, n1 = 0, n2 = 0, n3 = 0;
-         double       w0 = 0.0, w1 = 0.0, w2 = 0.0, w3 = 0.0;
-         if (k + 4 < len) { n0 = __ldcs(cp + q); w0 = __ldcs(vp + q); }
-         if (k + 5 < len) { n1 = __ldcs(cp + q + 32); w1 = __ldcs(vp + q + 32); }
-         if (k + 6 < len) { n2 = __ldcs(cp + q + 64); w2 = __ldcs(vp + q + 64); }
-         if (k + 7 < len) { n3 = __ldcs(cp + q + 96); w3 = __ldcs(vp + q + 96); }
-         const double p0 = __dmul_rn(v0, x0), p1 = __dmul_rn(v1, x1), p2 = __dmul_rn(v2, x2), p3 = __dmul_rn(v3, x3);
-         acc = __dadd_rn(acc, SUB ? -p0 : p0);
-         if (k + 1 < len) acc = __dadd_rn(acc, SUB ? -p1 : p1);
-         if (k + 2 < len) acc = __dadd_rn(acc, SUB ? -p2 : p2);
-         if (k + 3 < len) acc = __dadd_rn(acc, SUB ? -p3 : p3);
-         c0 = n0; c1 = n1; c2 = n2; c3 = n3;
-         v0 = w0; v1 = w1; v2 = w2; v3 = w3;
+         for (size_t h = base, he = base + len; h < he; h += 4)
+         {
+            const int4   o  = __ldg(reinterpret_cast<const int4 *>(a.sl_col + h));
+            const double x0 = LDX(a.x + (r + o.x));
+            const double x1 = (h + 1 < he) ? LDX(a.x + (r + o.y)) : 0.0;
+            const double x2 = (h + 2 < he) ? LDX(a.x + (r + o.z)) : 0.0;
+            const double x3 = (h + 3 < he) ? LDX(a.x + (r + o.w)) : 0.0;
+            const double p0 = __dmul_rn(__ldg(a.sl_val + h), x0);
+            acc = __dadd_rn(acc, SUB ? -p0 : p0);
+            if (h + 1 < he) { const double p1 = __dmul_rn(__ldg(a.sl_val + h + 1), x1); acc = __dadd_rn(acc, SUB ? -p1 : p1); }
+            if (h + 2 < he) { const double p2 = __dmul_rn(__ldg(a.sl_val + h + 2), x2); acc = __dadd_rn(acc, SUB ? -p2 : p2); }
+            if (h + 3 < he) { const double p3 = __dmul_rn(__ldg(a.sl_val + h + 3), x3); acc = __dadd_rn(acc, SUB ? -p3 : p3); }
+         }
+      }
+      else
+      {
+         const int    *cp = a.sl_col + base + ln;
+         const double *vp = a.sl_val + base + ln;
+         int    c0 = 0, c1 = 0, c2 = 0, c3 = 0;
+         double v0 = 0.0, v1 = 0.0, v2 = 0.0, v3 = 0.0;
+         if (0 < len) { c0 = __ldcs(cp); v0 = __ldcs(vp); }
+         if (1 < len) { c1 = __ldcs(cp + 32); v1 = __ldcs(vp + 32); }
+         if (2 < len) { c2 = __ldcs(cp + 64); v2 = __ldcs(vp + 64); }
+         if (3 < len) { c3 = __ldcs(cp + 96); v3 = __ldcs(vp + 96); }
+#pragma unroll 1
+         for (int k = 0; k < len; k += 4)
+         {
+            const double x0 = LDX(a.x + c0), x1 = LDX(a.x + c1), x2 = LDX(a.x + c2), x3 = LDX(a.x + c3);
+            const size_t q  = (size_t)(k + 4) * 32;
+            int          n0 = 0, n1 = 0, n2 = 0, n3 = 0;
+            double       w0 = 0.0, w1 = 0.0, w2 = 0.0, w3 = 0.0;
+            if (k + 4 < len) { n0 = __ldcs(cp + q); w0 = __ldcs(vp + q); }
+            if (k + 5 < len) { n1 = __ldcs(cp + q + 32); w1 = __ldcs(vp + q + 32); }
+            if (k + 6 < len) { n2 = __ldcs(cp + q + 64); w2 = __ldcs(vp + q + 64); }
+            if (k + 7 < len) { n3 = __ldcs(cp + q + 96); w3 = __ldcs(vp + q + 96); }
+            const double p0 = __dmul_rn(v0, x0), p1 = __dmul_rn(v1, x1), p2 = __dmul_rn(v2, x2), p3 = __dmul_rn(v3, x3);
+            acc = __dadd_rn(acc, SUB ? -p0 : p0);
+            if (k + 1 < len) acc = __dadd_rn(acc, SUB ? -p1 : p1);
+            if (k + 2 < len) acc = __dadd_rn(acc, SUB ? -p2 : p2);
+            if (k + 3 < len) acc = __dadd_rn(acc, SUB ? -p3 : p3);
+            c0 = n0; c1 = n1; c2 = n2; c3 = n3;
+            v0 = w0; v1 = w1; v2 = w2; v3 = w3;
+         }
       }
       if (OFFD && (meta & SELL_OFFD_BIT))
       {
@@ -468,8 +487,10 @@
       }
       if (valid)
       {
-         if (LATE && DIAG) o.d = a.d[r];
-         if (LATE && XOLD) o.xo = a.x[r];
+         if (DIAG) o.d = a.d[r];
+         if (XOLD) o.xo = a.x[r];
+         if (MODE == SPMV_AXPBY) o.yo = a.y[r];
+
          if (DOT) o.dv = a.dotv[r];
          if (MODE == SPMV_ADD) acc = __dadd_rn(a.y[r], acc);
          double yn = store_out<MODE, EXP>(a, r, row_epilogue<MODE>(a, o, acc), o.d, o.xo, nexp);
@@ -489,7 +510,7 @@
 __global__ void __launch_bounds__(SELL_T) k_spmv_sell(SpmvDev a) { sell_body<MODE, DOT, OFFD, EXP>(a); }
 
 __global__ void k_sell_meta(const int *rowptr, int nrows, int nslice, int *meta, int *width, int *max_slice_nnz,
-                            const int *offd_rowptr)
+                            const int *offd_rowptr, unsigned long long *padded)
 {
    const int lane = threadIdx.x & 31;
    const int s    = blockIdx.x * (blockDim.x >> 5) + (threadIdx.x >> 5);
@@ -505,35 +526,32 @@
       w = kj > w ? kj : w;
    }
    const int ob = (offd_rowptr && r < nrows && offd_rowptr[r + 1] > offd_rowptr[r]) ? SELL_OFFD_BIT : 0;
-   meta[(size_t)s * 32 + rank] = (len << 6) | lane | ob;
+   meta[(size_t)s * 32 + rank] = (len << SELL_LEN_SHIFT) | lane | ob;
    if (lane == 0)
    {
       width[s] = w;
       int hi   = s * 32 + 32;
       if (hi > nrows) hi = nrows;
       atomicMax(max_slice_nnz, rowptr[hi] - rowptr[s * 32]);
+      atomicAdd(padded, (unsigned long long)w);
    }
 }
 
 template <bool SORT>
-__global__ void k_sell_fill(const int *rowptr, const int *col, const double *val, int nrows, int nslice, const int *sl_off,
-                            const int *meta, int *scol, double *sval, int cap)
-{
-   extern __shared__ __align__(16) unsigned char sm_raw[];
-   const int lane = threadIdx.x & 31, w = threadIdx.x >> 5, nw = blockDim.x >> 5;
-   double   *vs = reinterpret_cast<double *>(sm_raw) + (size_t)w * cap;
-   int      *cs = reinterpret_cast<int *>(sm_raw + (size_t)nw * cap * sizeof(double)) + (size_t)w * cap;
-   const int s  = blockIdx.x * nw + w;
-   if (s >= nslice) return;
-   int hi = s * 32 + 32;
+__device__ __forceinline__ int sell_stage(const int *rowptr, const int *col, const double *val, int nrows, int s,
+                                          const int *meta, int *cs, double *vs, int &r, int &len)
+{
+   const int lane = threadIdx.x & 31;
+   int       hi   = s * 32 + 32;
    if (hi > nrows) hi = nrows;
    const int k0 = rowptr[s * 32], k1 = rowptr[hi];
    for (int k = k0 + lane; k < k1; k += 32) { cs[k - k0] = col[k]; vs[k - k0] = val[k]; }
    __syncwarp();
-   const int m = meta[(size_t)s * 32 + lane], len = m >> 6, r = s * 32 + (m & 31);
-   if (r >= nrows || len == 0) return;
-   const int rs = rowptr[r] - k0;
-   if (SORT)
+   const int m = meta[(size_t)s * 32 + lane];
+   len = m >> SELL_LEN_SHIFT;
+   r   = s * 32 + (m & 31);
+   const int rs = (r < nrows) ? rowptr[r] - k0 : 0;
+   if (SORT && len > 0)
    {
       const int b = rs + ((cs[rs] == r) ? 1 : 0), e = rs + len;
       for (int k = b + 1; k < e; ++k)
@@ -545,11 +563,77 @@
          cs[j + 1] = c; vs[j + 1] = v;
       }
    }
-   const size_t base = (size_t)sl_off[s] * 32 + lane;
+   __syncwarp();
+   return rs;
+}
+
+__device__ __forceinline__ int sell_stage_bufs(int cap, int *&cs, double *&vs)
+{
+   extern __shared__ __align__(16) unsigned char sm_raw[];
+   const int wi = threadIdx.x >> 5, nw = blockDim.x >> 5;
+   vs = reinterpret_cast<double *>(sm_raw) + (size_t)wi * cap;
+   cs = reinterpret_cast<int *>(sm_raw + (size_t)nw * cap * sizeof(double)) + (size_t)wi * cap;
+   return blockIdx.x * nw + wi;
+}
+
+template <bool SORT>
+__global__ void k_sell_class(const int *rowptr, const int *col, const double *val, int nrows, int nslice, int *meta,
+                             int *width, unsigned long long *census, int cap)
+{
+   int      *cs;
+   double   *vs;
+   const int s = sell_stage_bufs(cap, cs, vs), lane = threadIdx.x & 31;
+   if (s >= nslice) return;
+   int       r, len;
+   const int rs  = sell_stage<SORT>(rowptr, col, val, nrows, s, meta, cs, vs, r, len);
+   const int w   = __shfl_sync(0xffffffffu, len, 0);
+   const int r0  = __shfl_sync(0xffffffffu, r, 0);
+   const int rs0 = __shfl_sync(0xffffffffu, rs, 0);
+   bool      same = true;
+   for (int k = 0; k < len && same; ++k)
+      same = cs[rs + k] - r == cs[rs0 + k] - r0 && __double_as_longlong(vs[rs + k]) == __double_as_longlong(vs[rs0 + k]);
+   const bool stencil = __all_sync(0xffffffffu, same) && w > 0;
+   if (stencil) meta[(size_t)s * 32 + lane] |= SELL_STENCIL_BIT;
+   int total = len;
+   for (int o = 16; o > 0; o >>= 1) total += __shfl_xor_sync(0xffffffffu, total, o);
+   if (lane == 0)
+   {
+      if (stencil)
+      {
+         width[s] = (w + 31) / 32;
+         atomicAdd(&census[0], 1ull);
+         atomicAdd(&census[1], (unsigned long long)w);
+      }
+      else atomicAdd(&census[2], (unsigned long long)total);
+   }
+}
+
+template <bool SORT>
+__global__ void k_sell_fill(const int *rowptr, const int *col, const double *val, int nrows, int nslice, const int *sl_off,
+                            const int *meta, int *scol, double *sval, int cap)
+{
+   int      *cs;
+   double   *vs;
+   const int s = sell_stage_bufs(cap, cs, vs), lane = threadIdx.x & 31;
+   if (s >= nslice) return;
+   int          r, len;
+   const int    rs   = sell_stage<SORT>(rowptr, col, val, nrows, s, meta, cs, vs, r, len);
+   const size_t base = (size_t)sl_off[s] * 32;
+   if (meta[(size_t)s * 32] & SELL_STENCIL_BIT)
+   {
+      const int w = __shfl_sync(0xffffffffu, len, 0), r0 = __shfl_sync(0xffffffffu, r, 0);
+      const int rs0 = __shfl_sync(0xffffffffu, rs, 0);
+      for (int k = lane; k < ((w + 31) & ~31); k += 32)
+      {
+         scol[base + k] = k < w ? cs[rs0 + k] - r0 : 0;
+         sval[base + k] = k < w ? vs[rs0 + k] : 0.0;
+      }
+      return;
+   }
    for (int k = 0; k < len; ++k)
    {
-      scol[base + (size_t)k * 32] = cs[rs + k];
-      sval[base + (size_t)k * 32] = vs[rs + k];
+      scol[base + lane + (size_t)k * 32] = cs[rs + k];
+      sval[base + lane + (size_t)k * 32] = vs[rs + k];
    }
 }
 
@@ -741,6 +825,7 @@
 {
    dfree(A.sl_off); dfree(A.sl_meta); dfree(A.sl_col); dfree(A.sl_val);
    A.sl_off = A.sl_meta = A.sl_col = nullptr; A.sl_val = nullptr; A.nslice = 0;
+   A.sl_stencil = 0; A.sl_stencil_seg = A.sl_plain_nnz = 0;
 }
 
 static int sell_build(DevCSR &A)
@@ -748,49 +833,86 @@
    const bool sort = tunables().sell_sort != 0.0 && A.coarse_op;
    const int ns = cdiv(A.nrows, 32);
    int      *width = nullptr, *dmax = reinterpret_cast<int *>(g.dscal + S_TMP3);
+   unsigned long long *cnt = nullptr;
    HDK_TRY(dalloc(&A.sl_meta, (size_t)ns * 32));
    HDK_TRY(dalloc(&A.sl_off, (size_t)ns + 1));
    HDK_TRY(dalloc(&width, (size_t)ns + 1));
+   HDK_TRY(dalloc(&cnt, 4));
    HDK_CUDA(cudaMemsetAsync(width + ns, 0, sizeof(int), g.stream));
    HDK_CUDA(cudaMemsetAsync(dmax, 0, sizeof(int), g.stream));
+   HDK_CUDA(cudaMemsetAsync(cnt, 0, 4 * sizeof(unsigned long long), g.stream));
    static int fuse_on = -1;
    if (fuse_on < 0) { const char *e = getenv("HDK_FUSE_OFFD"); fuse_on = (e && atoi(e) == 0) ? 0 : 1; }
    const int *orp = fuse_on ? A.offd_rowptr : nullptr;
-   k_sell_meta<<<cdiv(ns, 8), 256, 0, g.stream>>>(A.rowptr, A.nrows, ns, A.sl_meta, width, dmax, orp);
+   k_sell_meta<<<cdiv(ns, 8), 256, 0, g.stream>>>(A.rowptr, A.nrows, ns, A.sl_meta, width, dmax, orp, cnt + 3);
    A.sl_offd_flags = (orp != nullptr);
    HDK_LAUNCH_CHECK();
+   unsigned long long hc[4] = {0, 0, 0, 0};
+   int                hmax  = 0;
+   HDK_CUDA(cudaMemcpyAsync(&hc[3], cnt + 3, sizeof(unsigned long long), cudaMemcpyDeviceToHost, g.stream));
+   HDK_CUDA(cudaMemcpyAsync(&hmax, dmax, sizeof(int), cudaMemcpyDeviceToHost, g.stream));
+   HDK_CUDA(cudaStreamSynchronize(g.stream));
+   const int64_t padded = (int64_t)hc[3] * 32;
+   const int     cap    = (hmax + 3) & ~3;
+   int           nw     = 4;
+   while (nw > 1 && (size_t)nw * cap * 12 > 200 * 1024) nw >>= 1;
+   if (padded > 3 * (int64_t)A.nnz + 4096 || (size_t)nw * cap * 12 > 200 * 1024) { dfree(width); dfree(cnt); sell_free(A); return HDK_OK; }
+   const size_t smem    = (size_t)nw * cap * 12;
+   const bool   do_sort = sort && A.nrows == A.ncols;
+   const int    grid    = cdiv(ns, nw);
+   if (tunables().sell_stencil != 0.0)
+   {
+      if (do_sort)
+      {
+         HDK_CUDA(cudaFuncSetAttribute(k_sell_class<true>, cudaFuncAttributeMaxDynamicSharedMemorySize, 200 * 1024));
+         k_sell_class<true><<<grid, nw * 32, smem, g.stream>>>(A.rowptr, A.col, A.val, A.nrows, ns, A.sl_meta, width, cnt, cap);
+      }
+      else
+      {
+         HDK_CUDA(cudaFuncSetAttribute(k_sell_class<false>, cudaFuncAttributeMaxDynamicSharedMemorySize, 200 * 1024));
+         k_sell_class<false><<<grid, nw * 32, smem, g.stream>>>(A.rowptr, A.col, A.val, A.nrows, ns, A.sl_meta, width, cnt, cap);
+      }
+      HDK_LAUNCH_CHECK();
+   }
+   else hc[2] = (unsigned long long)A.nnz;
    HDK_TRY(exclusive_scan_int(width, A.sl_off, ns + 1));
-   int h[2] = {0, 0};
-   HDK_CUDA(cudaMemcpyAsync(&h[0], A.sl_off + ns, sizeof(int), cudaMemcpyDeviceToHost, g.stream));
-   HDK_CUDA(cudaMemcpyAsync(&h[1], dmax, sizeof(int), cudaMemcpyDeviceToHost, g.stream));
+   int units = 0;
+   HDK_CUDA(cudaMemcpyAsync(&units, A.sl_off + ns, sizeof(int), cudaMemcpyDeviceToHost, g.stream));
+   if (tunables().sell_stencil != 0.0)
+      HDK_CUDA(cudaMemcpyAsync(hc, cnt, 3 * sizeof(unsigned long long), cudaMemcpyDeviceToHost, g.stream));
    HDK_CUDA(cudaStreamSynchronize(g.stream));
    dfree(width);
-   const int64_t padded = (int64_t)h[0] * 32;
-   const int     cap    = (h[1] + 3) & ~3;
-   int           nw     = 4;
-   while (nw > 1 && (size_t)nw * cap * 12 > 200 * 1024) nw >>= 1;
-   if (padded > 3 * (int64_t)A.nnz + 4096 || (size_t)nw * cap * 12 > 200 * 1024) { sell_free(A); return HDK_OK; }
-   HDK_TRY(dalloc(&A.sl_col, (size_t)padded + 32));
-   HDK_TRY(dalloc(&A.sl_val, (size_t)padded + 32));
-   const size_t smem = (size_t)nw * cap * 12;
-   const bool   do_sort = sort && A.nrows == A.ncols;
+   dfree(cnt);
+   A.sl_stencil     = (int)hc[0];
+   A.sl_stencil_seg = (int64_t)hc[1];
+   A.sl_plain_nnz   = (int64_t)hc[2];
+   HDK_TRY(dalloc(&A.sl_col, (size_t)units * 32 + 32));
+   HDK_TRY(dalloc(&A.sl_val, (size_t)units * 32 + 32));
    if (do_sort)
    {
       HDK_CUDA(cudaFuncSetAttribute(k_sell_fill<true>, cudaFuncAttributeMaxDynamicSharedMemorySize, 200 * 1024));
-      k_sell_fill<true><<<cdiv(ns, nw), nw * 32, smem, g.stream>>>(A.rowptr, A.col, A.val, A.nrows, ns, A.sl_off, A.sl_meta,
-                                                                    A.sl_col, A.sl_val, cap);
+      k_sell_fill<true><<<grid, nw * 32, smem, g.stream>>>(A.rowptr, A.col, A.val, A.nrows, ns, A.sl_off, A.sl_meta,
+                                                           A.sl_col, A.sl_val, cap);
    }
    else
    {
       HDK_CUDA(cudaFuncSetAttribute(k_sell_fill<false>, cudaFuncAttributeMaxDynamicSharedMemorySize, 200 * 1024));
-      k_sell_fill<false><<<cdiv(ns, nw), nw * 32, smem, g.stream>>>(A.rowptr, A.col, A.val, A.nrows, ns, A.sl_off, A.sl_meta,
-                                                                     A.sl_col, A.sl_val, cap);
+      k_sell_fill<false><<<grid, nw * 32, smem, g.stream>>>(A.rowptr, A.col, A.val, A.nrows, ns, A.sl_off, A.sl_meta,
+                                                            A.sl_col, A.sl_val, cap);
    }
    HDK_LAUNCH_CHECK();
    A.nslice = ns;
    A.kind   = 2;
    return HDK_OK;
 }
+
+double csr_stream_bytes(const DevCSR &A)
+{
+   if (A.kind != 2) return 12.0 * A.nnz + 4.0 * (A.nrows + 1);
+   return 4.0 * 32 * A.nslice + 4.0 * (A.nslice + 1) + 12.0 * (double)(A.sl_stencil_seg + A.sl_plain_nnz);
+}
+
+double parcsr_stream_bytes(const hdk_csr_s &A) { return csr_stream_bytes(A.diag) + 12.0 * A.offd.nnz; }
 
 int csr_analyze(DevCSR &A)
 {
diff --git a/hypredrive_b200/hdk.py b/hypredrive_b200/hdk.py
--- a/hypredrive_b200/hdk.py
+++ b/hypredrive_b200/hdk.py
@@ -67,6 +67,7 @@
         L.hdk_csr_matvec.argtypes = [C.c_void_p, C.c_double, C.c_void_p, C.c_double, C.c_void_p]
         L.hdk_csr_residual.argtypes = [C.c_void_p, C.c_void_p, C.c_void_p, C.c_void_p]
         L.hdk_csr_spmv_kind.argtypes = [C.c_void_p, C.POINTER(C.c_int), C.POINTER(C.c_double), C.POINTER(C.c_int)]
+        L.hdk_csr_sell_census.argtypes = [C.c_void_p, C.POINTER(C.c_int64), C.POINTER(C.c_int64), C.POINTER(C.c_double)]
         L.hdk_amg_default_params.argtypes = [C.POINTER(AmgParams)]
         L.hdk_amg_setup.argtypes = [C.c_void_p, C.POINTER(AmgParams), C.POINTER(C.c_void_p)]
         L.hdk_amg_destroy.argtypes = [C.c_void_p]
@@ -200,6 +201,11 @@
         check(lib().hdk_csr_spmv_kind(self.h, C.byref(k), C.byref(a), C.byref(m)))
         return dict(kind=k.value, avg_row=a.value, max_row=m.value)
 
+    def sell_census(self):
+        st, pl, by = C.c_int64(), C.c_int64(), C.c_double()
+        check(lib().hdk_csr_sell_census(self.h, C.byref(st), C.byref(pl), C.byref(by)))
+        return dict(stencil=st.value, plain=pl.value, bytes=by.value)
+
     def free(self):
         if self.h:
             lib().hdk_csr_destroy(self.h)
diff --git a/include/hdk.h b/include/hdk.h
--- a/include/hdk.h
+++ b/include/hdk.h
@@ -64,6 +64,7 @@
 int hdk_csr_matvec(const hdk_csr *A, double alpha, const double *x_d, double beta, double *y_d);
 int hdk_csr_residual(const hdk_csr *A, const double *x_d, const double *b_d, double *r_d);
 int hdk_csr_spmv_kind(const hdk_csr *A, int *kind, double *avg_row, int *max_row);
+int hdk_csr_sell_census(const hdk_csr *A, int64_t *stencil, int64_t *plain, double *bytes);
 
 int hdk_csr_stencil(int kind, int nx, int ny, int nz, const double c[3], int64_t row_start,
                     int64_t row_end, hdk_csr **A, double *b_d);
```
